# td-kwj-zp2023/webgpu-msm-bls12-377

Hardware: AMD Instinct MI355X
Metric: ms per 2^20 BLS12-377 G1 MSM (lower is better)
Workload: dtype u32 (29-bit limbs, 64-bit accumulate)

## Files before the change

include/msm377.h:

```cpp
#ifndef MSM377_H
#define MSM377_H

#include <stdint.h>

#ifdef __cplusplus
extern "C" {
#endif

#define MSM377_OK 0
#define MSM377_EINVAL (-1)
#define MSM377_EHIP (-2)
#define MSM377_ESCALAR (-3)
#define MSM377_ENOMEM (-4)
#define MSM377_ESTATE (-5)
#define MSM377_EGLVRANGE (-6)
#define MSM377_EEXCEPTIONAL (-7)
#define MSM377_EPOINT (-8)

#define MSM377_NUM_WINDOWS 16
#define MSM377_WINDOW_BITS 16
#define MSM377_G1_PARTIAL_POINTS 16
#define MSM377_G1_POINT_WORDS 48
#define MSM377_G1_WINDOW_PARTIAL_BYTES (MSM377_G1_PARTIAL_POINTS * MSM377_G1_POINT_WORDS * 4)

// ... 141 lines not shown
int msm377_g1_read_mul_table(msm377_ctx* ctx, uint32_t which, uint32_t index, msm377_mul_table_info* info, uint64_t first, uint64_t count, uint32_t* words);

int msm377_g1_xyzz_to_affine(const uint32_t xyzz[52], uint8_t out_xy[96]);

int msm377_ctx_set_glv(msm377_ctx* ctx, int mode);

int msm377_ctx_set_g1_form(msm377_ctx* ctx, int form);

int msm377_ctx_set_narrow_max(msm377_ctx* ctx, uint64_t max_points);

#define MSM377_FB_ACCUMULATE 4
#define MSM377_FB_MERGE 8
#define MSM377_FB_TREE 16
#define MSM377_FB_TAIL 32
#define MSM377_FB_CONVERT 64
int msm377_ctx_get_fallback_info(const msm377_ctx* ctx, uint64_t* count, uint32_t* last_mask);


int msm377_g1_batch_mul_device(msm377_ctx* ctx, const uint8_t base_xy[96], const void* d_scalars, uint64_t n, uint32_t out_form, void* d_out_points, uint8_t* d_out_inf);
int msm377_g1_batch_mul(msm377_ctx* ctx, const uint8_t base_xy[96], const uint8_t* scalars, uint64_t n, uint32_t out_form, uint8_t* out_points, uint8_t* out_inf);
int msm377_g1_batch_mul_host(const uint8_t base_xy[96], const uint8_t* scalars, uint64_t n, uint32_t out_form, uint8_t* out_points, uint8_t* out_inf);
int msm377_ctx_set_mul_window(msm377_ctx* ctx, int window_bits);
int msm377_ctx_get_last_mul_window(const msm377_ctx* ctx);
uint64_t msm377_ctx_get_mul_table_builds(const msm377_ctx* ctx);


#define MSM377_MUL_MAX_BASES 16
int msm377_g1_batch_mul_multi_device(msm377_ctx* ctx, const uint8_t* bases_xy , uint32_t k, const void* d_scalars, uint64_t n, uint64_t out_stride,
                                     uint64_t base_stride, uint32_t out_form, void* d_out_points, uint8_t* d_out_inf);
int msm377_g1_batch_mul_multi(msm377_ctx* ctx, const uint8_t* bases_xy, uint32_t k, const uint8_t* scalars, uint64_t n, uint64_t out_stride, uint64_t base_stride,
                              uint32_t out_form, uint8_t* out_points, uint8_t* out_inf);
int msm377_g1_batch_mul_multi_host(const uint8_t* bases_xy, uint32_t k, const uint8_t* scalars, uint64_t n, uint64_t out_stride, uint64_t base_stride, uint32_t out_form,
                                   uint8_t* out_points, uint8_t* out_inf);
uint64_t msm377_ctx_get_mul_multi_table_builds(const msm377_ctx* ctx);


int msm377_ed_batch_mul_multi_device(msm377_ctx* ctx, const uint8_t* bases_xy , uint32_t k, const void* d_scalars, uint64_t n, uint64_t out_stride,
                                     uint64_t base_stride, void* d_out_points);
int msm377_ed_batch_mul_multi(msm377_ctx* ctx, const uint8_t* bases_xy, uint32_t k, const uint8_t* scalars, uint64_t n, uint64_t out_stride, uint64_t base_stride,
                              uint8_t* out_points);
int msm377_ed_batch_mul_multi_host(const uint8_t* bases_xy, uint32_t k, const uint8_t* scalars, uint64_t n, uint64_t out_stride, uint64_t base_stride, uint8_t* out_points);
uint64_t msm377_ed_ctx_get_mul_table_builds(const msm377_ctx* ctx);
int msm377_ed_read_mul_table(msm377_ctx* ctx, uint32_t index, msm377_mul_table_info* info, uint64_t first, uint64_t count, uint32_t* words);


int msm377_g1_batch_mul_var_device(msm377_ctx* ctx, const void* d_points, const void* d_scalars, uint64_t n, uint32_t scalar_stride, uint32_t out_form, void* d_out_points,
                                   uint8_t* d_out_inf);
int msm377_g1_batch_mul_var(msm377_ctx* ctx, const uint8_t* points, const uint8_t* scalars, uint64_t n, uint32_t scalar_stride, uint32_t out_form, uint8_t* out_points,
                            uint8_t* out_inf);
int msm377_g1_batch_mul_var_host(const uint8_t* points, uint32_t point_form, const uint8_t* scalars, uint32_t scalar_form, uint64_t n, uint32_t scalar_stride,
                                 uint32_t out_form, uint8_t* out_points, uint8_t* out_inf);


int msm377_g1_batch_lincomb2_device(msm377_ctx* ctx, const void* d_p, const void* d_q, const void* d_a, const void* d_b, uint64_t n, uint32_t a_stride, uint32_t b_stride,
                                    uint32_t out_form, void* d_out_points, uint8_t* d_out_inf);
int msm377_g1_batch_lincomb2(msm377_ctx* ctx, const uint8_t* p, const uint8_t* q, const uint8_t* a, const uint8_t* b, uint64_t n, uint32_t a_stride, uint32_t b_stride,
                             uint32_t out_form, uint8_t* out_points, uint8_t* out_inf);
int msm377_g1_batch_lincomb2_host(const uint8_t* p, const uint8_t* q, uint32_t point_form, const uint8_t* a, const uint8_t* b, uint32_t scalar_form, uint64_t n, uint32_t a_stride,
                                  uint32_t b_stride, uint32_t out_form, uint8_t* out_points, uint8_t* out_inf);


#define MSM377_GEN_MAX      4096
#define MSM377_GEN_WIDE_MAX   64
int msm377_g1_set_generators(msm377_ctx* ctx, const uint8_t* gens_xy , uint32_t k, int window_bits);
int msm377_ctx_get_generators(const msm377_ctx* ctx, uint32_t* k, int* window_bits);
int msm377_g1_commit_rows_device(msm377_ctx* ctx, const void* d_scalars, uint64_t n, uint32_t k, uint64_t out_stride, uint64_t base_stride, uint32_t out_form, void* d_out_points,
                                 uint8_t* d_out_inf);
int msm377_g1_commit_rows(msm377_ctx* ctx, const uint8_t* scalars, uint64_t n, uint32_t k, uint64_t out_stride, uint64_t base_stride, uint32_t out_form, uint8_t* out_points,
                          uint8_t* out_inf);
int msm377_g1_commit_rows_host(const uint8_t* gens_xy, uint32_t k, const uint8_t* scalars, uint32_t scalar_form, uint64_t n, uint64_t out_stride, uint64_t base_stride,
                               uint32_t out_form, uint8_t* out_points, uint8_t* out_inf);
void msm377_commit_rows_plan(uint32_t k, uint32_t* segments, uint32_t* bases_per_segment, uint64_t* rows_per_pass);


#define MSM377_STAGE_CONVERT 0
#define MSM377_STAGE_DECOMPOSE 1
#define MSM377_STAGE_SORT 2
#define MSM377_STAGE_ACCUMULATE 3
#define MSM377_STAGE_REDUCE 4
#define MSM377_STAGE_TAIL 5
#define MSM377_STAGE_ACC_KERNEL 6
#define MSM377_NUM_STAGES 7
int msm377_ctx_set_timing(msm377_ctx* ctx, int enabled);
int msm377_ctx_get_stage_ms(msm377_ctx* ctx, double* ms_out);
int msm377_ctx_get_products_per_addition(const msm377_ctx* ctx);

#ifdef __cplusplus
}
#endif
#endif
```

webgpu-msm-bls12-377_amd/csrc/capi.hip:

```cpp
#include <hip/hip_runtime.h>
#include <stdlib.h>
#include <string.h>

#include <algorithm>

#include "context.hpp"
#include "host_tail.hpp"
#include "sequencer.hpp"
#include "batch_mul_host.hpp"
#include "batch_mul_multi_host.hpp"
#include "ed_batch_mul_host.hpp"
#include "commit_rows_host.hpp"
#include "commit_rows_plan.hpp"
#include "batch_lincomb2_host.hpp"
#include "batch_mul_var_host.hpp"
#include "import_host.hpp"
#include "validate_host.hpp"

using namespace msm377;


extern "C" {

const char* msm377_version(void) { return "msm377 0.1 gfx950"; }
// ... 292 lines not shown
  return batch_lincomb2_host(p, q, point_form, a, b, scalar_form, n, a_stride, b_stride, out_form, out_points, out_inf);
}

int msm377_ctx_set_mul_window(msm377_ctx* ctx, int window_bits) {
  if (!ctx || (window_bits != 0 && !batch_mul_width_supported(window_bits))) return MSM377_EINVAL;
  ctx->bm.window = window_bits;
  return MSM377_OK;
}

int msm377_ctx_get_last_mul_window(const msm377_ctx* ctx) { return ctx ? ctx->bm.last_window : 0; }

uint64_t msm377_ctx_get_mul_table_builds(const msm377_ctx* ctx) { return ctx ? ctx->bm.builds : 0; }

uint64_t msm377_ctx_get_mul_multi_table_builds(const msm377_ctx* ctx) { return ctx ? ctx->bmm.builds : 0; }

int msm377_ed_batch_mul_multi_host(const uint8_t* bases_xy, uint32_t k, const uint8_t* scalars, uint64_t n, uint64_t out_stride, uint64_t base_stride, uint8_t* out_points) {
  return ed_batch_mul_multi_host(bases_xy, k, scalars, n, out_stride, base_stride, out_points);
}

uint64_t msm377_ed_ctx_get_mul_table_builds(const msm377_ctx* ctx) { return ctx ? ctx->edbm.builds : 0; }

int msm377_ctx_get_last_check(const msm377_ctx* ctx, msm377_check_report* out) {
  if (!ctx || !out) return MSM377_EINVAL;
  *out = ctx->last_check;
  return MSM377_OK;
}

static int check_host_args(const uint8_t* points, uint64_t n, uint32_t flags, msm377_check_report* out) {
  return (!out || !check_flags_normal(flags) || (n && !points)) ? MSM377_EINVAL : MSM377_OK;
}
int msm377_g1_check_points_host(const uint8_t* points, uint64_t n, uint32_t flags, msm377_check_report* out) {
  if (check_host_args(points, n, flags, out)) return MSM377_EINVAL;
  check_points_host<G1HostCheck>(points, n, check_flags_normal(flags), out);
  return MSM377_OK;
}
int msm377_ed_check_points_host(const uint8_t* points, uint64_t n, uint32_t flags, msm377_check_report* out) {
  if (check_host_args(points, n, flags, out)) return MSM377_EINVAL;
  check_points_host<EdHostCheck>(points, n, check_flags_normal(flags), out);
  return MSM377_OK;
}

uint32_t msm377_short_windows(uint32_t scalar_bits, uint32_t bucket_log) {
  if (scalar_bits < 1 || scalar_bits > 253 || bucket_log < 1 || bucket_log > 15) return 0;
  return short_windows(scalar_bits, bucket_log);
}

int msm377_scalars_width_host(const uint8_t* scalars, uint64_t n, uint32_t scalar_bytes, uint32_t* bits_out) {
  if (!bits_out || (n && !scalars) || (scalar_bytes != 4 && scalar_bytes != 8 && scalar_bytes != 16 && scalar_bytes != 32)) return MSM377_EINVAL;
  uint32_t best = 0;
  for (uint64_t i = 0; i < n; i++) {
    const uint8_t* k = scalars + i * scalar_bytes;
    for (uint32_t j = scalar_bytes; j-- > 0;) {
      if (!k[j]) continue;
      const uint32_t len = 8 * j + 32 - (uint32_t)__builtin_clz((uint32_t)k[j]);
      best = std::max(best, len);
      break;
    }
  }
  *bits_out = best;
  return MSM377_OK;
}

int msm377_ctx_get_last_geometry(const msm377_ctx* ctx, uint32_t* windows, uint32_t* bucket_log) {
  if (!ctx) return MSM377_EINVAL;
  if (windows) *windows = ctx->last.geom_windows;
  if (bucket_log) *bucket_log = ctx->last.geom_log;
  return MSM377_OK;
}

uint32_t msm377_ctx_get_last_sort_elem_bytes(const msm377_ctx* ctx) { return ctx ? ctx->last.sort_elem : 0u; }

int msm377_ctx_set_narrow_max(msm377_ctx* ctx, uint64_t max_points) {
  if (!ctx) return MSM377_EINVAL;
  ctx->knobs.narrow_max_points = max_points;
  return MSM377_OK;
}

int msm377_ctx_set_timing(msm377_ctx* ctx, int enabled) {
  if (!ctx) return MSM377_EINVAL;
  ctx->timing = enabled == 2 ? 2 : (enabled != 0);
  return MSM377_OK;
}

int msm377_ctx_get_stage_ms(msm377_ctx* ctx, double* ms_out) {
  if (!ctx || !ms_out) return MSM377_EINVAL;
  for (int s = 0; s < MSM377_NUM_STAGES; s++) ms_out[s] = ctx->last.stage_ms[s];
  return MSM377_OK;
}

static int ed_wire_only(msm377_ctx* ctx) {
  if (!ctx || (ctx->point_form == MSM377_POINTS_WIRE && ctx->scalar_form == MSM377_SCALARS_WIRE)) return MSM377_OK;
  ctx->err = "the Edwards-BLS12 calls take the wire format only (msm377_ctx_set_input_format)";
  return MSM377_EINVAL;
}
int msm377_ctx_reserve_host_staging(msm377_ctx* ctx) { return eng::reserve_host_staging(ctx); }
int msm377_g1_msm_device(msm377_ctx* ctx, const void* d_points, const void* d_scalars, uint64_t n, uint8_t out_xy[96]) { return converted(ctx, eng::g1_msm_device(ctx, d_points, d_scalars, n, out_xy)); }
int msm377_g1_msm(msm377_ctx* ctx, const uint8_t* points, const uint8_t* scalars, uint64_t n, uint8_t out_xy[96]) { return converted(ctx, eng::g1_msm(ctx, points, scalars, n, out_xy)); }
int msm377_g1_msm_short_device(msm377_ctx* ctx, const void* d_points, const void* d_scalars, uint64_t n, uint32_t scalar_bytes, uint32_t scalar_bits, uint8_t out_xy[96]) { return converted(ctx, eng::g1_msm_short_device(ctx, d_points, d_scalars, n, scalar_bytes, scalar_bits, out_xy)); }
int msm377_g1_msm_short(msm377_ctx* ctx, const uint8_t* points, const uint8_t* scalars, uint64_t n, uint32_t scalar_bytes, uint32_t scalar_bits, uint8_t out_xy[96]) { return converted(ctx, eng::g1_msm_short(ctx, points, scalars, n, scalar_bytes, scalar_bits, out_xy)); }
int msm377_g1_msm_fixed_base_short_device(msm377_ctx* ctx, const void* d_scalars, uint64_t n, uint32_t scalar_bytes, uint32_t scalar_bits, uint8_t out_xy[96]) { return eng::g1_msm_fixed_base_short_device(ctx, d_scalars, n, scalar_bytes, scalar_bits, out_xy); }
int msm377_scalars_width_device(msm377_ctx* ctx, const void* d_scalars, uint64_t n, uint32_t scalar_bytes, uint32_t* bits_out) { return eng::scalars_width_device(ctx, d_scalars, n, scalar_bytes, bits_out); }
int msm377_ed_msm_device(msm377_ctx* ctx, const void* d_points, const void* d_scalars, uint64_t n, uint8_t out_xy[64]) { return converted(ctx, ed_wire_only(ctx) ? MSM377_EINVAL : eng::ed_msm_device(ctx, d_points, d_scalars, n, out_xy)); }
int msm377_ed_msm(msm377_ctx* ctx, const uint8_t* points, const uint8_t* scalars, uint64_t n, uint8_t out_xy[64]) { return converted(ctx, ed_wire_only(ctx) ? MSM377_EINVAL : eng::ed_msm(ctx, points, scalars, n, out_xy)); }
int msm377_ed_generate_bases_device(msm377_ctx* ctx, uint64_t seed, uint64_t n, void* d_points_out) { return ed_wire_only(ctx) ? MSM377_EINVAL : eng::ed_generate_bases_device(ctx, seed, n, d_points_out); }
int msm377_ed_batch_mul_multi_device(msm377_ctx* ctx, const uint8_t* bases_xy, uint32_t k, const void* d_scalars, uint64_t n, uint64_t out_stride, uint64_t base_stride,
                                     void* d_out_points) {
  return ed_wire_only(ctx) ? MSM377_EINVAL : eng::ed_batch_mul_multi_device(ctx, bases_xy, k, d_scalars, n, out_stride, base_stride, d_out_points);
}
int msm377_ed_batch_mul_multi(msm377_ctx* ctx, const uint8_t* bases_xy, uint32_t k, const uint8_t* scalars, uint64_t n, uint64_t out_stride, uint64_t base_stride, uint8_t* out_points) {
  return ed_wire_only(ctx) ? MSM377_EINVAL : eng::ed_batch_mul_multi(ctx, bases_xy, k, scalars, n, out_stride, base_stride, out_points);
}
int msm377_ed_read_mul_table(msm377_ctx* ctx, uint32_t index, msm377_mul_table_info* info, uint64_t first, uint64_t count, uint32_t* words) {
  return eng::ed_read_mul_table(ctx, index, info, first, count, words);
}
int msm377_g1_set_bases_device(msm377_ctx* ctx, const void* d_points, uint64_t n) { return converted(ctx, eng::g1_set_bases_device(ctx, d_points, n)); }
int msm377_g1_set_bases(msm377_ctx* ctx, const uint8_t* points, uint64_t n) { return converted(ctx, eng::g1_set_bases(ctx, points, n)); }
int msm377_g1_set_bases_precomputed_device(msm377_ctx* ctx, const void* d_points, uint64_t n) { return converted(ctx, eng::g1_set_bases_precomputed_device(ctx, d_points, n)); }
int msm377_g1_set_bases_precomputed(msm377_ctx* ctx, const uint8_t* points, uint64_t n) { return converted(ctx, eng::g1_set_bases_precomputed(ctx, points, n)); }
int msm377_g1_msm_fixed_base_device(msm377_ctx* ctx, const void* d_scalars, uint64_t n, uint8_t out_xy[96]) { return eng::g1_msm_fixed_base_device(ctx, d_scalars, n, out_xy); }
int msm377_g1_msm_fixed_base_batch_device(msm377_ctx* ctx, const void* d_scalars, uint64_t n, uint32_t batch, uint8_t* out_xy) { return eng::g1_msm_fixed_base_batch_device(ctx, d_scalars, n, batch, out_xy); }
int msm377_g1_msm_fixed_base(msm377_ctx* ctx, const uint8_t* scalars, uint64_t n, uint8_t out_xy[96]) { return eng::g1_msm_fixed_base(ctx, scalars, n, out_xy); }
int msm377_g1_glv_window_partials_device(msm377_ctx* ctx, const void* d_points, const void* d_scalars, uint64_t n, uint32_t win_begin, uint32_t win_count, uint8_t* partials_out) { return converted(ctx, eng::g1_glv_window_partials_device(ctx, d_points, d_scalars, n, win_begin, win_count, partials_out)); }
int msm377_g1_generate_bases_device(msm377_ctx* ctx, uint64_t seed, uint64_t n, void* d_points_out) { return eng::g1_generate_bases_device(ctx, seed, n, d_points_out); }
int msm377_g1_batch_mul_device(msm377_ctx* ctx, const uint8_t base_xy[96], const void* d_scalars, uint64_t n, uint32_t out_form, void* d_out_points, uint8_t* d_out_inf) { return eng::g1_batch_mul_device(ctx, base_xy, d_scalars, n, out_form, d_out_points, d_out_inf); }
int msm377_g1_batch_mul(msm377_ctx* ctx, const uint8_t base_xy[96], const uint8_t* scalars, uint64_t n, uint32_t out_form, uint8_t* out_points, uint8_t* out_inf) { return eng::g1_batch_mul(ctx, base_xy, scalars, n, out_form, out_points, out_inf); }
int msm377_g1_batch_mul_multi_device(msm377_ctx* ctx, const uint8_t* bases_xy, uint32_t k, const void* d_scalars, uint64_t n, uint64_t out_stride, uint64_t base_stride,
                                     uint32_t out_form, void* d_out_points, uint8_t* d_out_inf) {
  return eng::g1_batch_mul_multi_device(ctx, bases_xy, k, d_scalars, n, out_stride, base_stride, out_form, d_out_points, d_out_inf);
}
int msm377_g1_batch_mul_multi(msm377_ctx* ctx, const uint8_t* bases_xy, uint32_t k, const uint8_t* scalars, uint64_t n, uint64_t out_stride, uint64_t base_stride, uint32_t out_form,
                              uint8_t* out_points, uint8_t* out_inf) {
  return eng::g1_batch_mul_multi(ctx, bases_xy, k, scalars, n, out_stride, base_stride, out_form, out_points, out_inf);
}
int msm377_g1_set_generators(msm377_ctx* ctx, const uint8_t* gens_xy, uint32_t k, int window_bits) { return eng::g1_set_generators(ctx, gens_xy, k, window_bits); }
int msm377_g1_commit_rows_device(msm377_ctx* ctx, const void* d_scalars, uint64_t n, uint32_t k, uint64_t out_stride, uint64_t base_stride, uint32_t out_form, void* d_out_points,
                                 uint8_t* d_out_inf) {
  return eng::g1_commit_rows_device(ctx, d_scalars, n, k, out_stride, base_stride, out_form, d_out_points, d_out_inf);
}
int msm377_g1_commit_rows(msm377_ctx* ctx, const uint8_t* scalars, uint64_t n, uint32_t k, uint64_t out_stride, uint64_t base_stride, uint32_t out_form, uint8_t* out_points,
                          uint8_t* out_inf) {
  return eng::g1_commit_rows(ctx, scalars, n, k, out_stride, base_stride, out_form, out_points, out_inf);
}
int msm377_g1_batch_mul_var_device(msm377_ctx* ctx, const void* d_points, const void* d_scalars, uint64_t n, uint32_t scalar_stride, uint32_t out_form, void* d_out_points, uint8_t* d_out_inf) {
  return eng::g1_batch_mul_var_device(ctx, d_points, d_scalars, n, scalar_stride, out_form, d_out_points, d_out_inf);
}
int msm377_g1_batch_mul_var(msm377_ctx* ctx, const uint8_t* points, const uint8_t* scalars, uint64_t n, uint32_t scalar_stride, uint32_t out_form, uint8_t* out_points, uint8_t* out_inf) {
  return eng::g1_batch_mul_var(ctx, points, scalars, n, scalar_stride, out_form, out_points, out_inf);
}
int msm377_g1_batch_lincomb2_device(msm377_ctx* ctx, const void* d_p, const void* d_q, const void* d_a, const void* d_b, uint64_t n, uint32_t a_stride, uint32_t b_stride,
                                    uint32_t out_form, void* d_out_points, uint8_t* d_out_inf) {
  return eng::g1_batch_lincomb2_device(ctx, d_p, d_q, d_a, d_b, n, a_stride, b_stride, out_form, d_out_points, d_out_inf);
}
int msm377_g1_batch_lincomb2(msm377_ctx* ctx, const uint8_t* p, const uint8_t* q, const uint8_t* a, const uint8_t* b, uint64_t n, uint32_t a_stride, uint32_t b_stride,
                             uint32_t out_form, uint8_t* out_points, uint8_t* out_inf) {
  return eng::g1_batch_lincomb2(ctx, p, q, a, b, n, a_stride, b_stride, out_form, out_points, out_inf);
}
int msm377_g1_check_points_device(msm377_ctx* ctx, const void* d_points, uint64_t n, uint32_t flags, msm377_check_report* out) { return eng::g1_check_points_device(ctx, d_points, n, flags, out); }
int msm377_g1_check_points(msm377_ctx* ctx, const uint8_t* points, uint64_t n, uint32_t flags, msm377_check_report* out) { return eng::g1_check_points(ctx, points, n, flags, out); }
int msm377_ed_check_points_device(msm377_ctx* ctx, const void* d_points, uint64_t n, uint32_t flags, msm377_check_report* out) { return ed_wire_only(ctx) ? MSM377_EINVAL : eng::ed_check_points_device(ctx, d_points, n, flags, out); }
int msm377_ed_check_points(msm377_ctx* ctx, const uint8_t* points, uint64_t n, uint32_t flags, msm377_check_report* out) { return ed_wire_only(ctx) ? MSM377_EINVAL : eng::ed_check_points(ctx, points, n, flags, out); }

}
```

webgpu-msm-bls12-377_amd/csrc/common.hpp:

```cpp
#pragma once
#include <stdint.h>

#include "../../include/msm377.h"

#ifndef MSM_HD
#if defined(__HIPCC__)
#include <hip/hip_runtime.h>
#define MSM_HD __host__ __device__ __forceinline__
#else
#define MSM_HD inline __attribute__((always_inline))
#endif
#endif

namespace msm377 {

constexpr uint32_t NB = 32768;
constexpr uint32_t NBIN = NB + 1;
constexpr uint32_t RP = NBIN + 1;
constexpr uint32_t PT_WORDS = 52;
constexpr uint32_t BKT_WORDS = 64;
constexpr uint32_t MAX_SORT_BLOCKS = 256;
constexpr uint32_t TREE_LEVELS = 15;
constexpr uint32_t SEG_MIN = 16;
constexpr uint32_t SEG_MAX = 128;
constexpr uint32_t SEG_BINS = SEG_MAX + 1;
constexpr int ERR_SCALAR = 1, ERR_GLV_RANGE = 2, ERR_NARROW_RANGE = 128;
constexpr int ERR_SHORT_WIDTH = 256;
constexpr int ERR_TE_EXCEPTIONAL = MSM377_FB_ACCUMULATE, ERR_TE_MERGE = MSM377_FB_MERGE, ERR_TE_TREE = MSM377_FB_TREE, ERR_TE_CONVERT = MSM377_FB_CONVERT;
constexpr int ERR_TE_ANY = ERR_TE_EXCEPTIONAL | ERR_TE_MERGE | ERR_TE_TREE | ERR_TE_CONVERT;
constexpr uint32_t NARROW_LOG = 11;
constexpr uint32_t NARROW_SEG = 8;
constexpr uint32_t NARROW_EVEN_WINDOWS = 22, NARROW_EVEN_SIGNED = 11, NARROW_EVEN_BITS = NARROW_LOG + 1;
static_assert(NARROW_EVEN_SIGNED * NARROW_EVEN_BITS + (NARROW_EVEN_WINDOWS - NARROW_EVEN_SIGNED) * NARROW_LOG == 253, "the windows cover a 253-bit scalar");
constexpr uint32_t MAX_WINDOW_SLOTS = NARROW_EVEN_WINDOWS > MSM377_NUM_WINDOWS ? NARROW_EVEN_WINDOWS : MSM377_NUM_WINDOWS;

constexpr uint32_t short_windows(uint32_t bits, uint32_t L) { return bits / (L + 1) + 1; }
static_assert(short_windows(253, 15) == MSM377_NUM_WINDOWS && short_windows(253, NARROW_LOG) == NARROW_EVEN_WINDOWS, "at full width: the window counts of the main and the narrow path");

constexpr uint32_t NRANGE = 256;
constexpr uint32_t KRANGE = NB / NRANGE;
constexpr uint32_t KEY_TRACKED = 0x80000000u;
constexpr uint32_t KEY_UNSIGNED = 0x40000000u;
constexpr uint32_t SMALL_SORT_MAX = 1u << 16;
constexpr uint32_t SMALL_BINS_MAX = (1u << 12) + 1;
struct SortElem {
  uint32_t idx_sign;
  uint32_t key;
};
struct SortElem4 {
  uint32_t v;
};
constexpr uint32_t SORT_IDX_BITS = 23, SORT_SUB_BITS = 8;
constexpr uint64_t SORT_PACKED_MAX_COLUMNS = 1ull << SORT_IDX_BITS;
static_assert(SORT_IDX_BITS + SORT_SUB_BITS + 1 == 32, "index, sub and sign fill the 32-bit element");
static_assert(KRANGE < (1u << SORT_SUB_BITS), "sub = 0..KRANGE fits its field");
MSM_HD SortElem4 sort_pack(uint32_t idx, uint32_t sign, uint32_t sub) { return SortElem4{(sign << 31) | (sub << SORT_IDX_BITS) | idx}; }
MSM_HD uint32_t sort_sub(SortElem4 e) { return (e.v >> SORT_IDX_BITS) & ((1u << SORT_SUB_BITS) - 1u); }
MSM_HD uint32_t sort_idx_sign(SortElem4 e) { return e.v & ~(((1u << SORT_SUB_BITS) - 1u) << SORT_IDX_BITS); }
MSM_HD uint32_t range_first_key(uint32_t rg, uint32_t shift) { return rg * (KRANGE >> shift); }
inline uint32_t sort_elem_bytes(uint64_t columns, bool wide) { return (!wide && columns <= SORT_PACKED_MAX_COLUMNS) ? 4u : 8u; }

struct WorkItem {
  uint32_t row;
  uint32_t seg;
};
constexpr uint32_t META_BLOCK_WORDS = 2 * SEG_BINS + 4 + MSM377_NUM_WINDOWS;
constexpr size_t SLOT_WORDS = (size_t)MAX_WINDOW_SLOTS * MSM377_G1_PARTIAL_POINTS * MSM377_G1_POINT_WORDS;

constexpr uint32_t AFF_THREADS = 256, AFF_K = 8, AFF_BLOCK_POINTS = AFF_THREADS * AFF_K;
constexpr uint32_t AFF_STASH_WORDS = 52;
inline uint32_t affine_blocks(uint64_t n) { return (uint32_t)((n + AFF_BLOCK_POINTS - 1) / AFF_BLOCK_POINTS); }

constexpr uint32_t ACC_FLAG_WORD = 4;
constexpr uint32_t EVEN_FROM = 13;
constexpr uint32_t even_offset(uint32_t w) { return 16 * w - (w > EVEN_FROM ? w - EVEN_FROM : 0u); }
static_assert(even_offset(13) == 208 && even_offset(14) == 223 && even_offset(15) == 238 && even_offset(16) == 253, "13 x 16 + 3 x 15 = 253 bits");
constexpr uint32_t WIDE_BITS = MSM377_WIDE_WINDOW_BITS;
constexpr uint32_t WIDE_LOG = 19;
constexpr uint32_t WIDE_WINDOWS = 13;
constexpr uint32_t WIDE_FULL = 6;
constexpr uint32_t wide_width(uint32_t w) { return w < WIDE_FULL ? WIDE_BITS : WIDE_BITS - 1; }
constexpr uint32_t wide_offset(uint32_t w) { return w <= WIDE_FULL ? WIDE_BITS * w : WIDE_BITS * WIDE_FULL + (WIDE_BITS - 1) * (w - WIDE_FULL); }
static_assert(wide_offset(WIDE_WINDOWS - 1) == 234 && wide_offset(WIDE_WINDOWS - 1) + wide_width(WIDE_WINDOWS - 1) == 253, "the windows cover a 253-bit scalar");
constexpr uint32_t WIDE_NRANGE = 4096;
constexpr uint32_t WIDE_POINTS = WIDE_LOG + 1;
static_assert((1u << WIDE_LOG) == WIDE_NRANGE * KRANGE, "ranges of KRANGE keys cover the wide bucket set");
static_assert((1u << WIDE_LOG) <= MSM377_NUM_WINDOWS * NB, "the wide bucket set fits the main path's bucket, row and work-list buffers");
static_assert(WIDE_POINTS * 1 <= MAX_WINDOW_SLOTS * MSM377_G1_PARTIAL_POINTS, "the wide window record fits a partial-record slot");

constexpr uint32_t G1_REC_WORDS = 32;
constexpr uint32_t GLV_WINDOWS = MSM377_GLV_WINDOWS;

}
```

webgpu-msm-bls12-377_amd/csrc/context.hip:

```cpp
#include "context.hpp"

#include <string.h>

#include <algorithm>
#include <new>

#include "sequencer.hpp"

using namespace msm377;

hipError_t Resources::alloc(void** p, size_t bytes) {
  const hipError_t rc = hipMalloc(p, bytes);
  if (rc == hipSuccess) device.push_back(*p);
  else *p = nullptr;
  return rc;
}
hipError_t Resources::alloc_pinned(void** p, size_t bytes, unsigned flags) {
  const hipError_t rc = hipHostMalloc(p, bytes, flags);
  if (rc == hipSuccess) pinned.push_back(*p);
  else *p = nullptr;
  return rc;
}
hipError_t Resources::event(hipEvent_t* e, unsigned flags) {
  const hipError_t rc = hipEventCreateWithFlags(e, flags);
// ... 15 lines not shown
}
void Resources::release_all() {
  for (void* p : device) (void)hipFree(p);
  for (void* p : pinned) (void)hipHostFree(p);
  for (hipEvent_t e : events) (void)hipEventDestroy(e);
  for (auto s = streams.rbegin(); s != streams.rend(); ++s) (void)hipStreamDestroy(*s);
  *this = Resources();
}

bool WideBuffers::ensure(Resources& own, uint64_t n, size_t counts_words) {
  if (cap >= n) return true;
  release(own);
  if (own.alloc((void**)&digits, (size_t)WIDE_WINDOWS * n * 4) == hipSuccess && own.alloc((void**)&temp, (size_t)WIDE_WINDOWS * n * sizeof(SortElem)) == hipSuccess &&
      own.alloc((void**)&counts, counts_words * 4) == hipSuccess) {
    cap = n;
    return true;
  }
  release(own);
  (void)hipGetLastError();
  return false;
}
void WideBuffers::release(Resources& own) {
  for (void* p : {(void*)digits, (void*)temp, (void*)counts}) own.release(p);
  *this = WideBuffers();
}

namespace msm377 {
namespace eng {

int ctx_create(int device, uint64_t max_points, const Knobs& knobs, bool borrows_bases, msm377_ctx** out) {
  if (!out || max_points == 0 || max_points > (1ull << 30)) return MSM377_EINVAL;
  *out = nullptr;
  int count = 0;
  if (hipGetDeviceCount(&count) != hipSuccess || device < 0 || device >= count) return MSM377_EHIP;
  msm377_ctx* ctx = new (std::nothrow) msm377_ctx();
  if (!ctx) return MSM377_ENOMEM;
  ctx->device = device;
  ctx->cap = ctx->native.cap = max_points;
  ctx->knobs = knobs;
  ctx->tail_pool.wait_limit_ns = (int64_t)knobs.tail_wait_ms * 1000000ll;
  ctx->tail_pool.numa_local = knobs.tail_numa;
  Resources& own = ctx->own;
  const uint64_t cap = max_points;
  int prio_least = 0, prio_greatest = 0;
  bool ok = hipSetDevice(device) == hipSuccess;
  if (ok && hipDeviceGetStreamPriorityRange(&prio_least, &prio_greatest) != hipSuccess) prio_least = prio_greatest = 0;
  ok = ok && own.stream(&ctx->stream, &prio_greatest) == hipSuccess && own.stream(&ctx->stream2, &prio_least) == hipSuccess &&
       own.event(&ctx->bases_ready, hipEventDisableTiming) == hipSuccess;
  auto dalloc = [&](void** p, size_t bytes) { ok = ok && own.alloc(p, bytes) == hipSuccess; };
  if (!borrows_bases) dalloc((void**)&ctx->d_raw_points, cap * 96);
  dalloc((void**)&ctx->d_raw_scalars, cap * 32);
  if (!borrows_bases) dalloc((void**)&ctx->d_bases, 2 * cap * G1_REC_WORDS * 4);
  const uint64_t wcap = std::max<uint64_t>((uint64_t)MSM377_NUM_WINDOWS * cap, (uint64_t)NARROW_EVEN_WINDOWS * std::min<uint64_t>(cap, SMALL_SORT_MAX));
  dalloc((void**)&ctx->d_digits, wcap * 2);
  dalloc((void**)&ctx->d_range_counts, (size_t)NRANGE * MAX_SORT_BLOCKS * 4);
  dalloc((void**)&ctx->d_region_base, (size_t)MSM377_NUM_WINDOWS * (NRANGE + 1) * 4);
  dalloc((void**)&ctx->d_sort_temp, cap * MSM377_NUM_WINDOWS * sizeof(SortElem));
  dalloc((void**)&ctx->d_row_ptr, (size_t)MSM377_NUM_WINDOWS * RP * 4);
  dalloc((void**)&ctx->d_val_idx, wcap * 4);
  dalloc((void**)&ctx->d_buckets, (size_t)MSM377_NUM_WINDOWS * BKT_WORDS * NB * 4);
  dalloc((void**)&ctx->d_partials, (size_t)2 * SLOT_WORDS * 4);
  const uint64_t extra_items = std::max<uint64_t>((uint64_t)MSM377_NUM_WINDOWS * cap / SEG_MIN, (uint64_t)NARROW_EVEN_WINDOWS * std::min<uint64_t>(cap, SMALL_SORT_MAX) / NARROW_SEG) + 2;
  dalloc((void**)&ctx->d_work, ((size_t)MSM377_NUM_WINDOWS * NB + extra_items) * sizeof(WorkItem));
  dalloc((void**)&ctx->d_work_meta, (size_t)META_BLOCK_WORDS * 4);
  dalloc((void**)&ctx->d_row_ovf_base, (size_t)MSM377_NUM_WINDOWS * NB * 4);
  dalloc((void**)&ctx->d_split_rows, (size_t)MSM377_NUM_WINDOWS * NB * 4);
  dalloc((void**)&ctx->d_ovf, (size_t)extra_items * BKT_WORDS * 4);
  AffineConvert& aff = ctx->aff;
  ZeroCopyOut& zc = ctx->zc;
  const size_t aff_blocks = (size_t)affine_blocks(cap) + 1;
  dalloc((void**)&aff.d_count, 64);
  ok = ok && hipMemset(aff.d_count, 0, 64) == hipSuccess;
  dalloc((void**)&aff.d_stash, (size_t)affine_blocks(cap) * AFF_BLOCK_POINTS * AFF_STASH_WORDS * 4);
  dalloc((void**)&aff.d_trees, aff_blocks * 2 * AFF_THREADS * 13 * 4);
  const unsigned host_flags = hipHostMallocMapped | hipHostMallocCoherent;
  ok = ok && own.alloc_pinned((void**)&aff.h_prod, aff_blocks * 48, host_flags) == hipSuccess &&
       own.alloc_pinned((void**)&aff.h_inv, aff_blocks * 48, host_flags) == hipSuccess &&
       own.alloc_pinned((void**)&aff.h_flag, 64, host_flags) == hipSuccess &&
       hipHostGetDevicePointer((void**)&aff.dm_prod, aff.h_prod, 0) == hipSuccess &&
       hipHostGetDevicePointer((void**)&aff.dm_inv, aff.h_inv, 0) == hipSuccess &&
       hipHostGetDevicePointer((void**)&aff.dm_flag, aff.h_flag, 0) == hipSuccess &&
       own.event(&aff.up_done, hipEventDisableTiming) == hipSuccess;
  if (ok) aff.scratch.resize(aff_blocks);
  dalloc((void**)&ctx->d_err, 4 * sizeof(int));
  ok = ok && own.alloc_pinned((void**)&ctx->h_partials, (size_t)2 * SLOT_WORDS * 4, host_flags) == hipSuccess &&
       hipHostGetDevicePointer((void**)&zc.dm_partials, ctx->h_partials, 0) == hipSuccess &&
       own.alloc_pinned((void**)&zc.h_flag, 64, host_flags) == hipSuccess &&
       hipHostGetDevicePointer((void**)&zc.dm_flag, zc.h_flag, 0) == hipSuccess;
  if (ok) memset(zc.h_flag, 0, 64);
  dalloc((void**)&zc.d_count, 64);
  ok = ok && hipMemset(zc.d_count, 0, 64) == hipSuccess;
  ok = ok && own.alloc_pinned((void**)&ctx->h_err, 2 * sizeof(int)) == hipSuccess;
  for (int k = 0; ok && k < 2; k++) ok = ok && own.event(&ctx->done_ev[k], hipEventDisableTiming) == hipSuccess;
  for (int s = 0; ok && s < MSM377_NUM_STAGES; s++)
    for (int k = 0; k < 2; k++) ok = ok && own.event(&ctx->ev[s][k]) == hipSuccess;
  if (!ok) {
    ctx_destroy(ctx);
    return MSM377_ENOMEM;
  }
  *out = ctx;
  return MSM377_OK;
}

void ctx_destroy(msm377_ctx* ctx) {
  if (!ctx) return;
  ctx->tail_pool.shutdown();
  (void)hipSetDevice(ctx->device);
  if (ctx->stream) (void)hipStreamSynchronize(ctx->stream);
  if (ctx->stream2) (void)hipStreamSynchronize(ctx->stream2);
  if (ctx->twin) {
    twin_return(ctx);
    ctx_destroy(ctx->twin);
    ctx->twin = nullptr;
  }
  ctx->own.release_all();
  delete ctx;
}

int set_stage_capture(msm377_ctx* ctx, int enabled) {
  if (!ctx || enabled < 0 || enabled > 2) return MSM377_EINVAL;
  if (enabled && !ctx->d_buckets_snap) {
    HIP_TRY(ctx, hipSetDevice(ctx->device));
    if (ctx->own.alloc((void**)&ctx->d_buckets_snap, (size_t)MSM377_NUM_WINDOWS * BKT_WORDS * NB * 4) != hipSuccess) return MSM377_ENOMEM;
  }
  ctx->capture = enabled;
  ctx->last.stage.valid = false;
  return MSM377_OK;
}

int reserve_host_staging(msm377_ctx* ctx) {
  if (!ctx) return MSM377_EINVAL;
  HostStaging& st = ctx->staging;
  if (st.h_stage) return MSM377_OK;
  HIP_TRY(ctx, hipSetDevice(ctx->device));
  if (ctx->own.alloc_pinned((void**)&st.h_stage, (size_t)ctx->cap * 128) != hipSuccess) {
    ctx->err = "host staging buffer: out of pinned memory";
    return MSM377_ENOMEM;
  }
  for (int t = 0; t < 8; t++)
    if (!st.copy_stream[t]) HIP_TRY(ctx, ctx->own.stream(&st.copy_stream[t]));
  return MSM377_OK;
}

int ensure_import_buffers(msm377_ctx* ctx, bool host_staging) {
  NativeImport& nat = ctx->native;
  if (!nat.import_done) HIP_TRY(ctx, ctx->own.event(&nat.import_done, hipEventDisableTiming));
  if (!nat.d_inf_mask && ctx->own.alloc((void**)&nat.d_inf_mask, (2 * nat.mask_words() + 4) * 4) != hipSuccess) {
    (void)hipGetLastError();
    ctx->err = "native input forms: out of device memory";
    return MSM377_ENOMEM;
  }
  if (host_staging && !nat.d_native && ctx->own.alloc((void**)&nat.d_native, nat.points_bytes() + (size_t)ctx->cap * 32) != hipSuccess) {
    (void)hipGetLastError();
    ctx->err = "native input forms: out of device memory for the host-buffer staging";
    return MSM377_ENOMEM;
  }
  return MSM377_OK;
}

int bm_alloc(msm377_ctx* ctx, uint32_t** p, size_t bytes) {
  if (*p) return MSM377_OK;
  if (ctx->own.alloc((void**)p, bytes) != hipSuccess) {
    (void)hipGetLastError();
    ctx->err = "out of device memory for the batch multiplication scratch";
    return MSM377_ENOMEM;
  }
  return MSM377_OK;
}

}
}
```

webgpu-msm-bls12-377_amd/csrc/context.hpp:

```cpp
#pragma once
#include <hip/hip_runtime.h>

#include <functional>
#include <string>
#include <vector>

#include "common.hpp"
#include "fp64_host.hpp"
#include "knobs.hpp"
#include "tail_pool.hpp"

using msm377::SortElem;
using msm377::WorkItem;
using msm377::TailPool;
using msm377::Fp64;
using msm377::MAX_WINDOW_SLOTS;
using msm377::NARROW_SEG;
using msm377::Knobs;

struct Resources {
  std::vector<void*> device, pinned;
  std::vector<hipEvent_t> events;
  std::vector<hipStream_t> streams;
  hipError_t alloc(void** p, size_t bytes);
// ... 26 lines not shown
  int width = 0;
  uint32_t* table = nullptr;
  uint64_t table_cap = 0;
};

struct BatchMulState {
  int window = 0;
  int last_window = 0;
  uint64_t builds = 0;
  MulTableSlot single;
  uint32_t* stash = nullptr;
  uint32_t* trees = nullptr;
  uint32_t* block_prod = nullptr;
  uint32_t* block_inv = nullptr;
  uint32_t* row_bases = nullptr;
  uint32_t* base_wire = nullptr;
  uint32_t* var_table = nullptr;
};

struct BatchMulMultiState {
  MulTableSlot slot[MSM377_MUL_MAX_BASES];
  uint64_t builds = 0;
  uint32_t* row_bases = nullptr;
  uint32_t* bases_wire = nullptr;
};

struct EdBatchMulState {
  MulTableSlot slot[MSM377_MUL_MAX_BASES];
  uint64_t builds = 0;
};

struct GeneratorSet {
  uint32_t k = 0;
  int width = 0;
  uint32_t* tables = nullptr;
  bool valid() const { return k != 0; }
};

struct WideBuffers {
  uint32_t* digits = nullptr;
  SortElem* temp = nullptr;
  uint32_t* counts = nullptr;
  uint64_t cap = 0;
  bool ensure(Resources& own, uint64_t n, size_t counts_words);
  void release(Resources& own);
};

struct StageLayout {
  bool valid = false;
  msm377_stage_info info = {};
  const void* d_digits = nullptr;
  const uint32_t* d_key_max = nullptr;
  uint32_t coord_words = 16, limbs = 13;
};

struct BasesLayout {
  bool valid = false;
  msm377_bases_info info = {};
  const uint32_t* d_records = nullptr;
  const uint32_t* d_flagged = nullptr;
};


struct AffineConvert {
  uint32_t* d_stash = nullptr;
  uint32_t* d_trees = nullptr;
  uint32_t* h_prod = nullptr;
  uint32_t* h_inv = nullptr;
  uint32_t* h_flag = nullptr;
  uint32_t *dm_prod = nullptr, *dm_inv = nullptr, *dm_flag = nullptr;
  uint32_t* d_count = nullptr;
  hipEvent_t up_done = nullptr;
  std::vector<Fp64::El> scratch;
};

struct ZeroCopyOut {
  bool active = false;
  uint32_t out_seq = 0;
  uint32_t acc_seq = 0;
  uint32_t* h_flag = nullptr;
  uint32_t* dm_flag = nullptr;
  uint32_t* dm_partials = nullptr;
  uint32_t* d_count = nullptr;
};

struct NativeImport {
  uint64_t cap = 0;
  uint8_t* d_native = nullptr;
  uint32_t* d_inf_mask = nullptr;
  hipEvent_t import_done = nullptr;
  size_t mask_words() const { return (size_t)(((cap + 31) / 32 + 3) & ~3ull); }
  size_t points_bytes() const { return ((size_t)cap * 104 + 15) & ~(size_t)15; }
  uint8_t* native_points() const { return d_native; }
  uint8_t* native_scalars() const { return d_native + points_bytes(); }
};

struct HostStaging {
  uint8_t* h_stage = nullptr;
  hipStream_t copy_stream[8] = {};
};

struct LastCall {
  uint64_t n = 0;
  uint32_t geom_windows = 0, geom_log = 0;
  uint32_t sort_elem = 0;
  int form = -1;
  bool glv = false;
  int products = 0;
  double stage_ms[MSM377_NUM_STAGES] = {};
  StageLayout stage;
  BasesLayout bases;
};

struct Fallbacks {
  uint64_t count = 0;
  uint32_t mask = 0;
  uint64_t geometry_reruns = 0;
};

struct msm377_ctx {
  int device = 0;
  Resources own;
  Knobs knobs;
  hipStream_t stream = nullptr;
  hipStream_t stream2 = nullptr;
  hipEvent_t bases_ready = nullptr;
  uint64_t cap = 0;
  std::string err;
  uint32_t* d_raw_points = nullptr;
  uint32_t* d_raw_scalars = nullptr;
  uint32_t* d_bases = nullptr;
  uint16_t* d_digits = nullptr;
  uint32_t* d_range_counts = nullptr;
  uint32_t* d_region_base = nullptr;
  SortElem* d_sort_temp = nullptr;
  uint32_t* d_row_ptr = nullptr;
  uint32_t* d_val_idx = nullptr;
  uint32_t* d_buckets = nullptr;
  uint32_t* d_buckets_snap = nullptr;
  uint32_t* d_partials = nullptr;
  WorkItem* d_work = nullptr;
  uint32_t* d_work_meta = nullptr;
  uint32_t* d_row_ovf_base = nullptr;
  uint32_t* d_split_rows = nullptr;
  uint32_t* d_ovf = nullptr;
  int* d_err = nullptr;
  uint32_t* h_partials = nullptr;
  int* h_err = nullptr;
  hipEvent_t done_ev[2] = {};
  hipEvent_t ev[MSM377_NUM_STAGES][2] = {};
  uint32_t point_form = MSM377_POINTS_WIRE, scalar_form = MSM377_SCALARS_WIRE;
  int capture = 0;
  int timing = 0;
  ResidentBases resident;
  BatchMulState bm;
  BatchMulMultiState bmm;
  EdBatchMulState edbm;
  GeneratorSet gens;
  WideBuffers wide;
  AffineConvert aff;
  ZeroCopyOut zc;
  NativeImport native;
  HostStaging staging;
  LastCall last;
  Fallbacks fallback;
  msm377_check_report last_check = {0, 0, 0, 0, UINT64_MAX, 0, 0};
  std::function<int()> before_accumulate;
  TailPool tail_pool;
  msm377_ctx* twin = nullptr;
  bool twin_failed = false;
};

namespace msm377 {
namespace eng {

int ctx_create(int device, uint64_t max_points, const Knobs& knobs, bool borrows_bases, msm377_ctx** out);
void ctx_destroy(msm377_ctx* ctx);
int set_stage_capture(msm377_ctx* ctx, int enabled);
int reserve_host_staging(msm377_ctx* ctx);
int ensure_import_buffers(msm377_ctx* ctx, bool host_staging);
int bm_alloc(msm377_ctx* ctx, uint32_t** p, size_t bytes);

}
}
```

webgpu-msm-bls12-377_amd/csrc/kernels/accumulate.hpp:

```cpp
#pragma once
#include "../curves.hpp"
#include "reduce.hpp"

namespace msm377 {
namespace {



__device__ __forceinline__ const uint32_t* row_bounds(const uint32_t* __restrict__ row_ptr, uint32_t L, uint32_t ws, uint32_t t) {
  return row_ptr + (size_t)ws * ((1u << L) + 2) + t + 1;
}
__device__ __forceinline__ uint32_t row_len(const uint32_t* __restrict__ row_ptr, uint32_t L, uint32_t row) {
  const int at = (int)(row + 2 * (row >> L) + 1);
  return row_ptr[at + 1] - row_ptr[at];
}

struct RowSplit {
  uint32_t nseg, seglen, lastlen;
};
__device__ __forceinline__ RowSplit row_split(uint32_t len, uint32_t SEG) {
  RowSplit r;
  if (len <= SEG) {
    r.nseg = 1;
    r.seglen = r.lastlen = len;
    return r;
  }
  const uint32_t parts = (len + SEG - 1) / SEG;
  r.seglen = (len + parts - 1) / parts;
  r.nseg = (len + r.seglen - 1) / r.seglen;
  r.lastlen = len - (r.nseg - 1) * r.seglen;
  return r;
}

__global__ void __launch_bounds__(1024) k_work_hist(const uint32_t* __restrict__ row_ptr, uint32_t L, uint32_t rows, uint32_t SEG, uint32_t* __restrict__ work_hist,
                                                   uint32_t* __restrict__ row_ovf_base, uint32_t* __restrict__ counters ,
                                                   uint32_t* __restrict__ split_rows) {
  __shared__ uint32_t lh[SEG_BINS];
  __shared__ uint32_t blk[4];
  const uint32_t tid = threadIdx.x, row = blockIdx.x * 1024 + tid;
  if (tid < SEG_BINS) lh[tid] = 0;
  if (tid < 2) blk[tid] = 0;
  __syncthreads();
  RowSplit sp = {1, 0, 0};
  uint32_t my_split = 0, my_ovf = 0;
  if (row < rows) {
    sp = row_split(row_len(row_ptr, L, row), SEG);
    atomicAdd(&lh[sp.lastlen], 1u);
    if (sp.nseg > 1) {
      atomicAdd(&lh[sp.seglen], sp.nseg - 1);
      my_split = atomicAdd(&blk[0], 1u);
      my_ovf = atomicAdd(&blk[1], sp.nseg - 1);
    }
  }
  __syncthreads();
  if (tid < SEG_BINS && lh[tid]) atomicAdd(&work_hist[tid], lh[tid]);
  if (tid == 0 && blk[0]) {
    blk[2] = atomicAdd(&counters[0], blk[0]);
    blk[3] = atomicAdd(&counters[1], blk[1]);
  }
  __syncthreads();
  if (sp.nseg > 1) {
    row_ovf_base[row] = blk[3] + my_ovf;
    split_rows[blk[2] + my_split] = row;
  }
}

__global__ void __launch_bounds__(1024) k_work_scatter(const uint32_t* __restrict__ row_ptr, uint32_t L, uint32_t rows, uint32_t SEG,
                                                      const uint32_t* __restrict__ work_hist, uint32_t* __restrict__ cursor, uint32_t* __restrict__ total,
                                                      WorkItem* __restrict__ work) {
  __shared__ uint32_t lh[SEG_BINS];
  __shared__ uint32_t lbase[SEG_BINS];
  __shared__ uint32_t gh[SEG_BINS];
  const uint32_t tid = threadIdx.x, row = blockIdx.x * 1024 + tid;
  if (tid < SEG_BINS) {
    lh[tid] = 0;
    gh[tid] = work_hist[tid];
  }
  __syncthreads();
  uint32_t first = 0;
  if (tid < SEG_BINS) {
    for (uint32_t b = tid + 1; b < SEG_BINS; b++) first += gh[b];
    if (tid == 0 && blockIdx.x == 0) *total = first + gh[0];
  }
  RowSplit sp = {0, 0, 0};
  uint32_t rank_full = 0, rank_last = 0;
  if (row < rows) {
    sp = row_split(row_len(row_ptr, L, row), SEG);
    if (sp.nseg > 1) rank_full = atomicAdd(&lh[sp.seglen], sp.nseg - 1);
    rank_last = atomicAdd(&lh[sp.lastlen], 1u);
  }
  __syncthreads();
  if (tid < SEG_BINS && lh[tid]) lbase[tid] = first + atomicAdd(&cursor[tid], lh[tid]);
  __syncthreads();
  if (row < rows) {
    for (uint32_t s = 0; s + 1 < sp.nseg; s++) work[lbase[sp.seglen] + rank_full + s] = WorkItem{row, s};
    work[lbase[sp.lastlen] + rank_last] = WorkItem{row, sp.nseg - 1};
  }
}

template <class T>
__device__ __forceinline__ void pin_registers(T& o) {
  static_assert(sizeof(T) % 4 == 0, "whole words");
  uint32_t w[sizeof(T) / 4];
  __builtin_memcpy(w, &o, sizeof(T));
#pragma unroll
  for (int j = 0; j < (int)(sizeof(T) / 4); j++) asm volatile("" : "+v"(w[j]));
  __builtin_memcpy(&o, w, sizeof(T));
}

template <class CV, int OCC, class BP = CV, int PF = 0>
__global__ void __launch_bounds__(256, OCC) k_accumulate(const uint32_t* __restrict__ row_ptr, const uint32_t* __restrict__ val_idx,
                                                       const uint32_t* __restrict__ bases, uint32_t* __restrict__ buckets, uint64_t n,
                                                       const WorkItem* __restrict__ work, const uint32_t* __restrict__ work_total,
                                                       const uint32_t* __restrict__ row_ovf_base, uint32_t* __restrict__ ovf, uint32_t SEG,
                                                       int* __restrict__ err, const int* __restrict__ conv_err, uint32_t into, uint64_t table_stride, uint32_t L) {
  const uint32_t v = blockIdx.x * 256 + threadIdx.x;
  if (v == 0 && *conv_err) atomicOr(err, *conv_err);
  if (v >= *work_total) return;
  const WorkItem it = work[v];
  const uint32_t ws = it.row >> L, t = it.row & ((1u << L) - 1);
  const uint32_t* rb = row_bounds(row_ptr, L, ws, t);
  const uint32_t* vi = val_idx + (size_t)ws * n;
  bases += (size_t)ws * table_stride * BP::REC_WORDS;
  const uint32_t row_beg = rb[0], row_end = rb[1];
  const uint32_t seglen = row_split(row_end - row_beg, SEG).seglen;
  uint32_t k = row_beg + it.seg * seglen;
  const uint32_t end = (row_end - k > seglen) ? k + seglen : row_end;
  typename CV::Pt acc = (into && it.seg == 0) ? load_bucket<CV>(buckets, L, ws, t) : CV::identity();
  const bool start_fresh = !(into && it.seg == 0);
  bool bad = false;
  if (k < end) {
    static_assert(PF == 0, "one record in flight");
    uint32_t e_cur = vi[k];
    uint32_t e_nxt = (k + 1 < end) ? vi[k + 1] : 0u;
    typename BP::Base rec = BP::load_base(bases, e_cur & 0x7fffffffu);
    bool more = true;
    auto advance = [&]() {
      k++;
      more = k < end;
      if (more) {
        rec = BP::load_base(bases, e_nxt & 0x7fffffffu);
        e_cur = e_nxt;
        e_nxt = (k + 1 < end) ? vi[k + 1] : 0u;
      }
    };
    auto stage = [&](auto first_tag) {
      constexpr bool FIRST = decltype(first_tag)::value;
      const bool neg = (e_cur >> 31) != 0;
      if constexpr (FIRST) {
        const typename BP::Base cur = rec;
        advance();
        acc = BP::first(cur, neg);
      } else {
        typename BP::Ops ops = BP::signed_ops(rec, neg);
        pin_registers(ops);
        advance();
        acc = BP::madd(acc, ops);
      }
      bad |= CV::is_bad(acc);
    };
    if (start_fresh) stage(std::true_type{});
    while (more) stage(std::false_type{});
  }
  if (bad) atomicOr(err, ERR_TE_EXCEPTIONAL);
  if (it.seg == 0) {
    store_bucket<CV>(buckets, L, ws, t, acc);
  } else {
    store_record<CV>(ovf + (size_t)(row_ovf_base[it.row] + it.seg - 1) * CV::BKT_WORDS, acc);
  }
}

template <class F, class K>
__device__ __forceinline__ typename TeLazy<F, K>::Ext te_madd_quad(const typename TeLazy<F, K>::Ext& a, const typename F::El& mine, uint32_t q) {
  using El = typename F::El;
  const El m1 = F::mul_lz(sel4(q, F::add_kp_sub(a.y, K::KP2, a.x), F::add_lz(a.y, a.x), a.t, a.z), mine);
  const El pa = quad_bcast<0>(m1), pb = quad_bcast<1>(m1), c = quad_bcast<2>(m1), d = quad_bcast<3>(m1);
  const El e = F::norm(F::add_kp_sub(pb, K::KP2, pa)), f = F::norm(F::add_kp_sub(d, K::KP2, c));
  const El g = F::norm(F::add_lz(d, c)), h = F::add_lz(pb, pa);
  const El m3 = F::mul_lz(sel4(q, e, h, h, f), sel4(q, f, g, e, g));
  typename TeLazy<F, K>::Ext o;
  o.x = quad_bcast<0>(m3);
  o.y = quad_bcast<1>(m3);
  o.t = quad_bcast<2>(m3);
  o.z = quad_bcast<3>(m3);
  return o;
}

template <class CV>
__global__ void __launch_bounds__(256, 2) k_accumulate_quad(const uint32_t* __restrict__ row_ptr, const uint32_t* __restrict__ val_idx,
                                                          const uint32_t* __restrict__ bases, uint32_t* __restrict__ buckets, uint64_t n,
                                                          const WorkItem* __restrict__ work, const uint32_t* __restrict__ work_total,
                                                          const uint32_t* __restrict__ row_ovf_base, uint32_t* __restrict__ ovf, uint32_t SEG,
                                                          int* __restrict__ err, const int* __restrict__ conv_err, uint32_t into, uint32_t L) {
  using El = typename CV::F::El;
  using K = typename CV::Pt_K;
  const uint32_t gid = blockIdx.x * 256 + threadIdx.x;
  const uint32_t v = gid >> 2, q = threadIdx.x & 3;
  if (gid == 0 && *conv_err) atomicOr(err, *conv_err);
  if (v >= *work_total) return;
  const WorkItem it = work[v];
  const uint32_t ws = it.row >> L, t = it.row & ((1u << L) - 1);
  const uint32_t* rb = row_bounds(row_ptr, L, ws, t);
  const uint32_t* vi = val_idx + (size_t)ws * n;
  const uint32_t row_beg = rb[0], row_end = rb[1];
  const uint32_t seglen = row_split(row_end - row_beg, SEG).seglen;
  uint32_t k = row_beg + it.seg * seglen;
  const uint32_t end = (row_end - k > seglen) ? k + seglen : row_end;
  const bool continues = into && it.seg == 0;
  typename CV::Pt acc = continues ? load_bucket<CV>(buckets, L, ws, t) : CV::identity();
  bool bad = false;
  auto load_mine = [&](uint32_t e) {
    const bool neg = (e >> 31) != 0;
    const uint32_t comp = q < 2 ? (q ^ (neg ? 1u : 0u)) : q;
    const uint32_t* src = bases + (size_t)(e & 0x7fffffffu) * CV::REC_WORDS + comp * CV::NL;
    El r;
#pragma unroll
    for (int j = 0; j < (int)CV::NL; j++) r.l[j] = src[j];
    return r;
  };
  if (k < end && !continues) {
    const uint32_t e = vi[k];
    acc = CV::first(CV::load_base(bases, e & 0x7fffffffu), (e >> 31) != 0);
    bad |= CV::is_bad(acc);
    k++;
  }
  if (k < end) {
    uint32_t e_cur = vi[k];
    uint32_t e_nxt = (k + 1 < end) ? vi[k + 1] : 0u;
    El cur = load_mine(e_cur);
    for (;;) {
      k++;
      const bool more = k < end;
      El nxt = cur;
      uint32_t e_nn = 0u;
      if (more) {
        nxt = load_mine(e_nxt);
        if (k + 1 < end) e_nn = vi[k + 1];
      }
      const El mine = (q == 2 && (e_cur >> 31)) ? CV::F::kp_sub(K::KP2, cur) : cur;
      acc = te_madd_quad<typename CV::F, K>(acc, mine, q);
      bad |= CV::is_bad(acc);
      if (!more) break;
      cur = nxt;
      e_cur = e_nxt;
      e_nxt = e_nn;
    }
  }
  if (bad) atomicOr(err, ERR_TE_EXCEPTIONAL);
  uint32_t* dst = it.seg == 0 ? bucket_ptr<CV>(buckets, L, ws, t) : ovf + (size_t)(row_ovf_base[it.row] + it.seg - 1) * CV::BKT_WORDS;
  store_coord<CV>(dst + q * CV::COORD_WORDS, coord4(q, acc).l);
}

constexpr uint32_t OVF_FOLDED = 0x80000000u;
constexpr uint32_t LONG_ROW_PARTIALS = 32, FOLD_THREADS = 512, FOLD_BLOCKS = 64;
static_assert((1u << 15) <= FOLD_THREADS * FOLD_BLOCKS, "one pass of the grid sees every row of a window (L <= 15)");
template <class CV>
__global__ void __launch_bounds__(FOLD_THREADS) k_fold_long_rows(const uint32_t* __restrict__ row_ptr, uint32_t* __restrict__ row_ovf_base, uint32_t* __restrict__ ovf,
                                                                 uint32_t SEG, int* __restrict__ err, uint32_t L, uint32_t ws) {
  __shared__ uint32_t list[FOLD_THREADS];
  __shared__ uint32_t nlist;
  if (threadIdx.x == 0) nlist = 0;
  __syncthreads();
  {
    const uint32_t t = blockIdx.x + gridDim.x * threadIdx.x;
    if (t < (1u << L) && row_split(row_len(row_ptr, L, (ws << L) + t), SEG).nseg > LONG_ROW_PARTIALS) list[atomicAdd(&nlist, 1u)] = (ws << L) + t;
  }
  __syncthreads();
  const uint32_t q = threadIdx.x & 3, quad = threadIdx.x >> 2;
  bool bad = false;
  for (uint32_t i = 0; i < nlist; i++) {
    const uint32_t row = list[i];
    uint32_t* rec = ovf + (size_t)row_ovf_base[row] * CV::BKT_WORDS;
    for (uint32_t cur = row_split(row_len(row_ptr, L, row), SEG).nseg - 1; cur > 1;) {
      const uint32_t half = (cur + 1) / 2;
      for (uint32_t j = quad; j + half < cur; j += FOLD_THREADS / 4) {
        uint32_t* a = rec + (size_t)j * CV::BKT_WORDS;
        const typename CV::Pt sum = add_quad(load_record_quad<CV>(a, q), load_record_quad<CV>(rec + (size_t)(j + half) * CV::BKT_WORDS, q), q);
        bad |= CV::is_bad(sum);
        store_coord<CV>(a + q * CV::COORD_WORDS, coord4(q, sum).l);
      }
      cur = half;
      __syncthreads();
    }
  }
  __syncthreads();
  for (uint32_t i = threadIdx.x; i < nlist; i += FOLD_THREADS) row_ovf_base[list[i]] |= OVF_FOLDED;
  if (bad) atomicOr(err, ERR_TE_MERGE);
}

template <class CV>
__global__ void __launch_bounds__(256, 2) k_merge_split_rows_quad(const uint32_t* __restrict__ row_ptr, uint32_t* __restrict__ buckets,
                                                                  const uint32_t* __restrict__ counters, const uint32_t* __restrict__ split_rows,
                                                                  const uint32_t* __restrict__ row_ovf_base, const uint32_t* __restrict__ ovf, uint32_t SEG,
                                                                  int* __restrict__ err, uint32_t L, uint32_t* __restrict__ host_flag, uint32_t seq) {
  if (host_flag && blockIdx.x == 0 && threadIdx.x == 0) __hip_atomic_store(host_flag, seq, __ATOMIC_RELAXED, __HIP_MEMORY_SCOPE_SYSTEM);
  const uint32_t count = counters[0];
  const uint32_t q = threadIdx.x & 3;
  for (uint32_t i = (blockIdx.x * 256 + threadIdx.x) >> 2; i < count; i += gridDim.x * 64) {
    const uint32_t row = split_rows[i];
    const uint32_t len = row_len(row_ptr, L, row);
    const uint32_t ovf_at = row_ovf_base[row];
    const uint32_t nseg = (ovf_at & OVF_FOLDED) ? 2u : row_split(len, SEG).nseg;
    const uint32_t ws = row >> L, t = row & ((1u << L) - 1);
    typename CV::Pt acc = load_bucket_quad<CV>(buckets, L, ws, t, q);
    const uint32_t* src = ovf + (size_t)(ovf_at & ~OVF_FOLDED) * CV::BKT_WORDS;
    typename CV::Pt nxt = load_record_quad<CV>(src, q);
    bool bad = false;
    for (uint32_t s = 1; s < nseg; s++) {
      const typename CV::Pt cur = nxt;
      if (s + 1 < nseg) nxt = load_record_quad<CV>(src + (size_t)s * CV::BKT_WORDS, q);
      acc = add_quad(acc, cur, q);
      bad |= CV::is_bad(acc);
    }
    if (bad) atomicOr(err, ERR_TE_MERGE);
    const typename CV::F::El c = coord4(q, acc);
    store_coord<CV>(bucket_ptr<CV>(buckets, L, ws, t) + q * CV::COORD_WORDS, c.l);
  }
}

}
}
```

webgpu-msm-bls12-377_amd/csrc/kernels/sort.hpp:

```cpp
#pragma once
#include "../curves.hpp"
#include "decompose.hpp"

namespace msm377 {
namespace {



template <class F>
__device__ __forceinline__ void for_each_digit(const uint16_t* __restrict__ dg, uint64_t beg, uint64_t end, uint32_t tid, uint32_t nthreads, F f) {
  uint64_t head = beg;
  while (head < end && (((uintptr_t)(dg + head)) & 15)) head++;
  for (uint64_t i = beg + tid; i < head; i += nthreads) f(i, (uint32_t)dg[i]);
  const uint64_t groups = (end - head) / 8;
  const uint4* v = reinterpret_cast<const uint4*>(dg + head);
  for (uint64_t g = tid; g < groups; g += nthreads) {
    const uint4 q = v[g];
    const uint32_t w[4] = {q.x, q.y, q.z, q.w};
#pragma unroll
    for (int k = 0; k < 4; k++) {
      f(head + g * 8 + 2 * k, w[k] & 0xffffu);
      f(head + g * 8 + 2 * k + 1, w[k] >> 16);
    }
  }
// ... 88 lines not shown
    cnt[tid] = 0;
  }
  __syncthreads();
  const uint64_t beg = (uint64_t)c * per_chunk;
  const uint64_t end = (beg + per_chunk < n) ? beg + per_chunk : n;
  const uint16_t* dg = digits + (size_t)ws * n;
  E* out = temp + (size_t)ws * n;
  for (uint64_t tile0 = beg; tile0 < end; tile0 += PT_TILE) {
    const uint64_t i0 = tile0 + (uint64_t)tid * 8;
    uint32_t d[8];
    uint32_t valid = 0;
    if (i0 + 8 <= end && (((uintptr_t)(dg + i0)) & 15) == 0) {
      const uint4 q = *reinterpret_cast<const uint4*>(dg + i0);
      const uint32_t w[4] = {q.x, q.y, q.z, q.w};
#pragma unroll
      for (int k = 0; k < 4; k++) {
        d[2 * k] = w[k] & 0xffffu;
        d[2 * k + 1] = w[k] >> 16;
      }
      valid = 0xffu;
    } else {
#pragma unroll
      for (int j = 0; j < 8; j++) {
        d[j] = 0;
        if (i0 + j < end) {
          d[j] = dg[i0 + j];
          valid |= 1u << j;
        }
      }
    }
    uint32_t key[8], sign[8], rg[8], rk[8];
#pragma unroll
    for (int j = 0; j < 8; j++) {
      digit_key(d[j], uns, key[j], sign[j]);
      rg[j] = key_range(key[j], shift);
      rk[j] = 0;
      if ((valid >> j) & 1u) rk[j] = atomicAdd(&cnt[rg[j]], 1u);
    }
    __syncthreads();
    uint32_t mine = 0, incl = 0;
    if (tid < NRANGE) {
      mine = cnt[tid];
      incl = mine;
#pragma unroll
      for (int off = 1; off < 64; off <<= 1) {
        const uint32_t v = __shfl_up((int)incl, off, 64);
        if ((tid & 63) >= (uint32_t)off) incl += v;
      }
      if ((tid & 63) == 63) wsum[tid >> 6] = incl;
    }
    __syncthreads();
    if (tid < NRANGE) {
      uint32_t before = 0;
      for (uint32_t w = 0; w < (tid >> 6); w++) before += wsum[w];
      const uint32_t excl = before + incl - mine;
      toff[tid] = excl;
      gdelta[tid] = cur[tid] - excl;
      cur[tid] += mine;
      cnt[tid] = 0;
    }
    __syncthreads();
#pragma unroll
    for (int j = 0; j < 8; j++)
      if ((valid >> j) & 1u) {
        const uint32_t slot = toff[rg[j]] + rk[j];
        stage[slot] = Ops::make((uint32_t)(i0 + j), sign[j], key[j], rg[j], shift);
        if constexpr (Ops::TAGGED) tag[slot] = (uint8_t)rg[j];
      }
    __syncthreads();
    const uint32_t tile_len = (uint32_t)((end - tile0 < PT_TILE) ? end - tile0 : PT_TILE);
    for (uint32_t p = tid; p < tile_len; p += 1024) {
      const E e = stage[p];
      uint32_t range;
      if constexpr (Ops::TAGGED)
        range = tag[p];
      else
        range = key_range(e.key, shift);
      out[gdelta[range] + p] = e;
    }
    __syncthreads();
  }
}

constexpr uint32_t LS_CACHE = 6144;
constexpr uint32_t LS_REG = LS_CACHE / 256;
template <class E>
__global__ void __launch_bounds__(256) k_local_sort_lds(const E* __restrict__ temp, const uint32_t* __restrict__ region_base,
                                                        uint32_t* __restrict__ row_ptr, uint32_t* __restrict__ val_idx, uint64_t n,
                                                        const uint32_t* __restrict__ key_max, uint32_t NR, uint32_t NBK) {
  using Ops = ElemOps<E>;
  constexpr uint32_t NBINS = KRANGE + 1;
  static_assert(NBINS <= 256, "one bin per thread");
  __shared__ uint32_t bins[NBINS];
  __shared__ uint32_t part[256];
  __shared__ uint32_t sorted[LS_CACHE];
  const uint32_t RPW = NBK + 2;
  const uint32_t r = blockIdx.x, ws = blockIdx.y, tid = threadIdx.x;
  const uint32_t shift = key_max ? win_shift(key_max[ws]) : 0u;
  const uint32_t KR = KRANGE >> shift;
  const uint32_t lo = r * KR;
  const bool last = shift == 0 && r == NR - 1;
  const uint32_t nb = KR + (last ? 1u : 0u);
  const uint32_t rbeg = region_base[ws * (NR + 1) + r], rend = region_base[ws * (NR + 1) + r + 1];
  const uint32_t len = rend - rbeg;
  const bool cached = len <= LS_CACHE;
  const E* in = temp + (size_t)ws * n + rbeg;
  if (tid < NBINS) bins[tid] = 0;
  __syncthreads();
  E e[LS_REG];
  if (cached) {
#pragma unroll
    for (uint32_t u = 0; u < LS_REG; u++) {
      const uint32_t i = u * 256 + tid;
      e[u] = Ops::none(lo);
      if (i < len) e[u] = in[i];
    }
#pragma unroll
    for (uint32_t u = 0; u < LS_REG; u++)
      if (u * 256 + tid < len) atomicAdd(&bins[Ops::bin(e[u], lo)], 1u);
  } else {
    for (uint32_t i0 = 0; i0 < len; i0 += 2048) {
      E f[8];
#pragma unroll
      for (int u = 0; u < 8; u++) {
        const uint32_t i = i0 + u * 256 + tid;
        f[u] = Ops::none(lo);
        if (i < len) f[u] = in[i];
      }
#pragma unroll
      for (int u = 0; u < 8; u++)
        if (i0 + u * 256 + tid < len) atomicAdd(&bins[Ops::bin(f[u], lo)], 1u);
    }
  }
  __syncthreads();
  const uint32_t own = tid < nb ? bins[tid] : 0u;
  part[tid] = own;
  __syncthreads();
  for (uint32_t off = 1; off < 256; off <<= 1) {
    const uint32_t v = tid >= off ? part[tid - off] : 0u;
    __syncthreads();
    part[tid] += v;
    __syncthreads();
  }
  uint32_t* rp = row_ptr + (size_t)ws * RPW + lo;
  const uint32_t start = rbeg + part[tid] - own;
  __syncthreads();
  if (tid < nb) {
    bins[tid] = start;
    rp[tid] = start;
  }
  if (tid == 0 && last) rp[nb] = rend;
  if (shift) {
    const uint32_t covered = NR * KR, total = region_base[ws * (NR + 1) + NR];
    const uint32_t per_block = (RPW - covered + NR - 1) / NR;
    uint32_t* rp_w = row_ptr + (size_t)ws * RPW;
    for (uint32_t j = tid; j < per_block; j += 256) {
      const uint32_t idx = covered + r * per_block + j;
      if (idx < RPW) rp_w[idx] = total;
    }
  }
  __syncthreads();
  uint32_t* vi = val_idx + (size_t)ws * n;
  if (cached) {
#pragma unroll
    for (uint32_t u = 0; u < LS_REG; u++)
      if (u * 256 + tid < len) sorted[atomicAdd(&bins[Ops::bin(e[u], lo)], 1u) - rbeg] = Ops::idx_sign(e[u]);
    __syncthreads();
    for (uint32_t i = tid; i < len; i += 256) vi[rbeg + i] = sorted[i];
  } else {
    for (uint32_t i0 = 0; i0 < len; i0 += 2048) {
      E f[8];
#pragma unroll
      for (int u = 0; u < 8; u++) {
// ... 64 lines not shown
```

webgpu-msm-bls12-377_amd/csrc/knobs.hpp:

```cpp
#pragma once
#include <limits.h>
#include <stdint.h>
#include <stdlib.h>

#include <algorithm>
#include <type_traits>
#include <utility>

#include "common.hpp"
#include "tail_pool.hpp"
#include "validate_host.hpp"

namespace msm377 {

struct Knobs {
  int glv_mode = 0;
  int g1_form = 1;
  uint32_t conv_wave_prio = 1;
  int64_t aff_prewake_us = 600;
  uint32_t upload_chunks = 4;
  uint32_t upload_split_pct = 30;
  uint64_t upload_chunk_min = 1ull << 18;
  int tail_threads = 6;
  int tail_wait_ms = 2000;
  int64_t tail_spin_us = 1000;
  bool tail_trace = false;
  bool tail_numa = true;
  bool te_affine_msm = true;
  uint64_t narrow_max_points = 1ull << 16;
  int precomp_bits = MSM377_WINDOW_BITS;
  uint64_t affine_min_points = 1ull << 20;
  uint32_t seg_plain = 0, seg_glv = 0;
  int zc_out = 1;
  uint32_t narrow_seg = 0;
  uint64_t narrow_quad_items = 100000;
  uint32_t coop_threads = 131072;
  uint32_t narrow_tail_from = 4;
  bool tail_lds = true;
  bool reduce_columns = true;
  bool even_windows = true;
  uint32_t sort_elem = 8;
  bool twin_batches = true;
  uint32_t base_checks = 0;
  uint32_t tail_from = 7;

  static inline Knobs from_env();
};

namespace knob_rule {
template <auto F>
using field_t = std::remove_reference_t<decltype(std::declval<Knobs&>().*F)>;
template <auto F>
void flag(Knobs& k, const char* e) { k.*F = atoi(e) != 0; }
template <auto F>
void raw_int(Knobs& k, const char* e) { k.*F = (field_t<F>)atoi(e); }
template <auto F, int LO, int HI>
void int_in(Knobs& k, const char* e) { k.*F = (field_t<F>)std::min(std::max(atoi(e), LO), HI); }
template <auto F>
void u64(Knobs& k, const char* e) { k.*F = strtoull(e, nullptr, 10); }
template <auto F>
void i64(Knobs& k, const char* e) { k.*F = atoll(e); }
inline void wide_or_16(Knobs& k, const char* e) { k.precomp_bits = atoi(e) == (int)WIDE_BITS ? (int)WIDE_BITS : MSM377_WINDOW_BITS; }
inline void four_or_8(Knobs& k, const char* e) { k.sort_elem = atoi(e) == 4 ? 4u : 8u; }
inline void check_mask(Knobs& k, const char* e) { k.base_checks = check_flags_normal((uint32_t)strtoul(e, nullptr, 0)); }
}

inline Knobs Knobs::from_env() {
  using namespace knob_rule;
  static constexpr struct {
    const char* name;
    void (*rule)(Knobs&, const char*);
  } TABLE[] = {
      {"MSM377_GLV", raw_int<&Knobs::glv_mode>},
      {"MSM377_G1_FORM", flag<&Knobs::g1_form>},
      {"MSM377_CONV_WAVE_PRIO", flag<&Knobs::conv_wave_prio>},
      {"MSM377_AFF_PREWAKE_US", i64<&Knobs::aff_prewake_us>},
      {"MSM377_UPLOAD_CHUNKS", int_in<&Knobs::upload_chunks, 2, 7>},
      {"MSM377_UPLOAD_SPLIT", int_in<&Knobs::upload_split_pct, 5, 90>},
      {"MSM377_UPLOAD_CHUNK_MIN", u64<&Knobs::upload_chunk_min>},
      {"MSM377_TAIL_THREADS", int_in<&Knobs::tail_threads, 1, TailPool::WORKERS + 1>},
      {"MSM377_TAIL_WAIT_MS", int_in<&Knobs::tail_wait_ms, 1, INT_MAX>},
      {"MSM377_TAIL_SPIN_US", i64<&Knobs::tail_spin_us>},
      {"MSM377_TAIL_TRACE", flag<&Knobs::tail_trace>},
      {"MSM377_TAIL_NUMA", flag<&Knobs::tail_numa>},
      {"MSM377_TE_AFFINE_MSM", flag<&Knobs::te_affine_msm>},
      {"MSM377_NARROW_MAX", u64<&Knobs::narrow_max_points>},
      {"MSM377_PRECOMP_BITS", wide_or_16},
      {"MSM377_AFFINE_MIN", u64<&Knobs::affine_min_points>},
      {"MSM377_SEG_PLAIN", int_in<&Knobs::seg_plain, (int)SEG_MIN, (int)SEG_MAX>},
      {"MSM377_SEG_GLV", int_in<&Knobs::seg_glv, (int)SEG_MIN, (int)SEG_MAX>},
      {"MSM377_ZERO_COPY_OUT", raw_int<&Knobs::zc_out>},
      {"MSM377_NARROW_SEG", int_in<&Knobs::narrow_seg, (int)NARROW_SEG, (int)SEG_BINS - 1>},
      {"MSM377_NARROW_QUAD_ITEMS", u64<&Knobs::narrow_quad_items>},
      {"MSM377_COOP_THREADS", raw_int<&Knobs::coop_threads>},
      {"MSM377_NARROW_TAIL_FROM", int_in<&Knobs::narrow_tail_from, 1, (int)TREE_LEVELS>},
      {"MSM377_TAIL_LDS", flag<&Knobs::tail_lds>},
      {"MSM377_REDUCE_COLUMNS", flag<&Knobs::reduce_columns>},
      {"MSM377_EVEN_WINDOWS", flag<&Knobs::even_windows>},
      {"MSM377_SORT_ELEM", four_or_8},
      {"MSM377_TWIN_BATCH", flag<&Knobs::twin_batches>},
      {"MSM377_BASE_CHECKS", check_mask},
      {"MSM377_TAIL_FROM", int_in<&Knobs::tail_from, 1, (int)TREE_LEVELS>},
  };
  Knobs k;
  for (const auto& row : TABLE)
    if (const char* e = getenv(row.name)) row.rule(k, e);
  return k;
}

}
```

webgpu-msm-bls12-377_amd/csrc/sequencer.hip:

```cpp
#include "sequencer.hpp"

#include <hip/hip_runtime.h>
#include <string.h>

#include <algorithm>
#include <atomic>
#include <chrono>
#include <functional>
#include <initializer_list>
#include <thread>
#include <type_traits>
#include <vector>

#include "context.hpp"
#include "host_tail.hpp"
#include "ed_batch_mul_host.hpp"
#include "validate_host.hpp"
#include "kernels/accumulate.hpp"
#include "kernels/batch_mul.hpp"
#include "kernels/batch_mul_multi.hpp"
#include "kernels/ed_batch_mul.hpp"
#include "kernels/commit_rows.hpp"
#include "kernels/convert.hpp"
#include "kernels/decompose.hpp"
// ... 12 lines not shown
bool hip_ok(msm377_ctx* ctx, int hip_error, const char* what) {
  const hipError_t e = (hipError_t)hip_error;
  if (e == hipSuccess) return true;
  if (ctx) ctx->err = std::string(what) + ": " + hipGetErrorString(e);
  return false;
}

namespace {

void note_fallback(msm377_ctx* ctx, uint32_t mask) {
  ctx->fallback.count++;
  ctx->fallback.mask = mask;
}

struct HipFail {
  hipError_t e = hipSuccess;
  const char* what = "";
  int record(msm377_ctx* ctx, int rc) const {
    hip_ok(ctx, e, what);
    return rc;
  }
};
int h2d_staged(msm377_ctx* ctx, void* d_dst, const uint8_t* src, size_t bytes, size_t stage_off, HipFail* fail = nullptr) {
#define H2D_TRY(call)                \
  do {                               \
    const hipError_t e_ = (call);    \
    if (e_ != hipSuccess) {          \
      if (fail) *fail = {e_, #call}; \
      else hip_ok(ctx, e_, #call);   \
      return MSM377_EHIP;            \
    }                                \
  } while (0)
  constexpr int NT_MAX = 8;
  constexpr int NT = 4;
  constexpr size_t SMALL = 8u << 20, PIECE = 4u << 20;
  if (bytes < SMALL) {
    H2D_TRY(hipMemcpy(d_dst, src, bytes, hipMemcpyHostToDevice));
    return MSM377_OK;
  }
  if (!ctx->staging.h_stage && reserve_host_staging(ctx) != MSM377_OK) {
    (void)hipGetLastError();
    H2D_TRY(hipMemcpy(d_dst, src, bytes, hipMemcpyHostToDevice));
    return MSM377_OK;
  }
  size_t npieces = (bytes + PIECE - 1) / PIECE;
  npieces = (npieces + NT - 1) / NT * NT;
  const size_t piece = ((bytes + npieces - 1) / npieces + 4095) & ~(size_t)4095;
  uint8_t* stage = ctx->staging.h_stage + stage_off;
  hipError_t errs[NT_MAX + 1];
  std::thread workers[NT_MAX];
  const int device = ctx->device;
  std::atomic<size_t> next{0};
  auto copy_pieces = [&, device](int t) {
    hipError_t e = hipSetDevice(device);
    for (;;) {
      const size_t c = next.fetch_add(1, std::memory_order_relaxed);
      const size_t off = c * piece;
      if (c >= npieces || off >= bytes || e != hipSuccess) break;
      const size_t len = (bytes - off < piece) ? bytes - off : piece;
      memcpy(stage + off, src + off, len);
      e = hipMemcpyAsync((uint8_t*)d_dst + off, stage + off, len, hipMemcpyHostToDevice, ctx->staging.copy_stream[t]);
    }
    if (e == hipSuccess) e = hipStreamSynchronize(ctx->staging.copy_stream[t]);
    errs[t] = e;
  };
  for (int t = 0; t <= NT; t++) errs[t] = hipSuccess;
  for (int t = 0; t < NT; t++) workers[t] = std::thread([&copy_pieces, t] { copy_pieces(t); });
  copy_pieces(NT);
  for (int t = 0; t < NT; t++) workers[t].join();
  for (int t = 0; t <= NT; t++) H2D_TRY(errs[t]);
  return MSM377_OK;
#undef H2D_TRY
}

void identity_wire(uint8_t out[96]) {
  memset(out, 0, 96);
  out[48] = 1;
}

struct StageTimer {
  msm377_ctx* c;
  int s;
  hipStream_t st;
  bool on() const { return c->timing == 1 || (c->timing == 2 && s == MSM377_STAGE_ACC_KERNEL); }
  StageTimer(msm377_ctx* ctx, int stage, hipStream_t stream) : c(ctx), s(stage), st(stream) {
    if (on()) (void)hipEventRecord(c->ev[s][0], st);
  }
  ~StageTimer() {
    if (on()) (void)hipEventRecord(c->ev[s][1], st);
  }
};

void note_bases(msm377_ctx* ctx, uint32_t form, const uint32_t* d_records, uint64_t n, uint64_t first = 0, bool glv = false) {
  static const uint32_t REC[4] = {64, 40, 32, 32}, LIMBS[4] = {13, 13, 13, 9}, COORDS[4] = {4, 3, 2, 3};
  BasesLayout b;
  b.info.form = form;
  b.info.record_words = REC[form];
  b.info.limbs = LIMBS[form];
  b.info.coords = COORDS[form];
  b.info.n = first + n;
  b.info.windows = 1;
  b.info.glv = glv ? 1 : 0;
  b.info.window_stride = first + n;
  b.info.records = (glv ? 2 : 1) * (first + n);
  b.d_records = d_records;
  if (form != MSM377_BASES_ED && ctx->point_form == MSM377_POINTS_MONT_FLAG && ctx->native.d_inf_mask) b.d_flagged = ctx->native.d_inf_mask + 2 * ctx->native.mask_words();
  b.valid = true;
  ctx->last.bases = b;
}
template <class CV>
constexpr uint32_t bases_form_of() {
  return std::is_same<CV, TeDev>::value ? MSM377_BASES_TE_PROJECTIVE : std::is_same<CV, EdDev>::value ? MSM377_BASES_ED : MSM377_BASES_WEIERSTRASS;
}

template <class CV>
int convert_bases(msm377_ctx* ctx, const uint32_t* d_raw, uint64_t n, uint64_t first = 0, bool clear_err = true) {
  if (n == 0) return MSM377_OK;
  if (ctx->timing == 1) (void)hipEventRecord(ctx->ev[MSM377_STAGE_CONVERT][0], ctx->stream2);
  if (clear_err) hipLaunchKernelGGL(k_clear_words, dim3(1), dim3(256), 0, ctx->stream2, (uint32_t*)(ctx->d_err + 2), 1u, (uint32_t*)nullptr, 0u);
  hipLaunchKernelGGL(k_convert_bases<CV>, dim3((unsigned)((n + 255) / 256)), dim3(256), 0, ctx->stream2, d_raw, ctx->d_bases + first * CV::REC_WORDS, n,
                     ctx->d_err + 2);
  HIP_TRY(ctx, hipGetLastError());
  note_bases(ctx, bases_form_of<CV>(), ctx->d_bases, n, first);
  if (ctx->timing == 1) (void)hipEventRecord(ctx->ev[MSM377_STAGE_CONVERT][1], ctx->stream2);
  HIP_TRY(ctx, hipEventRecord(ctx->bases_ready, ctx->stream2));
  return MSM377_OK;
}

int affine_convert_begin(msm377_ctx* ctx, const uint32_t* d_raw, uint64_t n, const uint32_t* prev_window_records = nullptr, uint32_t doublings = 0,
                         bool clear_err = true) {
  if (n == 0) return MSM377_OK;
  const uint32_t nblk = affine_blocks(n);
  if (ctx->timing == 1) (void)hipEventRecord(ctx->ev[MSM377_STAGE_CONVERT][0], ctx->stream2);
  __atomic_store_n(ctx->aff.h_flag, 0u, __ATOMIC_RELEASE);
  if (clear_err) hipLaunchKernelGGL(k_clear_words, dim3(1), dim3(256), 0, ctx->stream2, (uint32_t*)(ctx->d_err + 2), 1u, (uint32_t*)nullptr, 0u);
  if (prev_window_records)
    hipLaunchKernelGGL(k_affine_up<AffDoublingSource>, dim3(nblk), dim3(AFF_THREADS), 0, ctx->stream2, AffDoublingSource{prev_window_records, doublings}, n,
                       ctx->aff.d_stash, ctx->aff.d_trees, ctx->aff.dm_prod, ctx->aff.dm_flag, ctx->aff.d_count, ctx->d_err + 2, ctx->knobs.conv_wave_prio);
  else
    hipLaunchKernelGGL(k_affine_up<AffWireSource>, dim3(nblk), dim3(AFF_THREADS), 0, ctx->stream2, AffWireSource{d_raw}, n, ctx->aff.d_stash, ctx->aff.d_trees,
                       ctx->aff.dm_prod, ctx->aff.dm_flag, ctx->aff.d_count, ctx->d_err + 2, ctx->knobs.conv_wave_prio);
  HIP_TRY(ctx, hipGetLastError());
  HIP_TRY(ctx, hipEventRecord(ctx->aff.up_done, ctx->stream2));
  if (ctx->knobs.tail_threads > 1 && nblk >= 32) ctx->tail_pool.prewake(ctx->knobs.aff_prewake_us, std::min(ctx->knobs.tail_threads, TailPool::WORKERS + 1) - 1);
  return MSM377_OK;
}

int affine_convert_finish(msm377_ctx* ctx, uint32_t* d_records_out, uint64_t n) {
  if (n == 0) return MSM377_OK;
  const uint32_t nblk = affine_blocks(n);
  const auto t0 = std::chrono::steady_clock::now();
  for (uint32_t spins = 0; __atomic_load_n(ctx->aff.h_flag, __ATOMIC_ACQUIRE) != nblk; spins++) {
    __builtin_ia32_pause();
    if ((spins & 0xfff) == 0xfff && std::chrono::steady_clock::now() - t0 > std::chrono::milliseconds(20)) {
      HIP_TRY(ctx, hipEventSynchronize(ctx->aff.up_done));
      break;
    }
  }
  if (__atomic_load_n(ctx->aff.h_flag, __ATOMIC_ACQUIRE) != nblk) {
    ctx->err = "batched affine conversion: the block products did not arrive";
    return MSM377_EHIP;
  }
  {
    const int inv_rc = invert_block_products_mt(ctx, 0, nblk);
    ctx->tail_pool.disarm();
    if (inv_rc) return inv_rc;
  }
  hipLaunchKernelGGL(k_affine_down, dim3(nblk), dim3(AFF_THREADS), 0, ctx->stream2, n, ctx->aff.d_stash, ctx->aff.d_trees, ctx->aff.dm_inv, d_records_out, ctx->knobs.conv_wave_prio);
// ... 41 lines not shown
  WindowPlan p = plan_equal16(tail);
  p.recode = RECODE_EVEN16;
  p.short_from = EVEN_FROM;
  return p;
}
WindowPlan plan_narrow22() {
  WindowPlan p = plan_equal16(TE_TAIL, NARROW_EVEN_WINDOWS);
  p.recode = RECODE_NARROW22;
  p.bucket_log = NARROW_LOG;
  p.short_from = NARROW_EVEN_SIGNED;
  return p;
}
WindowPlan folded_behind_table(WindowPlan p, const uint32_t* table, uint64_t stride) {
  p.table = table;
  p.table_stride = stride;
  p.records = 1;
  p.on_caller = true;
  return p;
}
WindowPlan plan_wide13(const uint32_t* table, uint64_t stride) {
  WindowPlan p = folded_behind_table(plan_equal16(TE_TAIL, 1), table, stride);
  p.recode = RECODE_WIDE13;
  p.bucket_log = WIDE_LOG;
  return p;
}
WindowPlan plan_glv8(uint32_t slots = GLV_WINDOWS) {
  WindowPlan p = plan_equal16(XYZZ_TAIL, slots);
  p.recode = RECODE_GLV8;
  p.on_caller = true;
  return p;
}
WindowPlan plan_short(TailKind tail, uint32_t bytes, uint32_t bits, bool narrow) {
  const uint32_t L = narrow ? NARROW_LOG : (uint32_t)MSM377_WINDOW_BITS - 1;
  WindowPlan p = plan_equal16(tail, short_windows(bits, L));
  p.recode = RECODE_SHORT;
  p.bucket_log = L;
  p.short_bytes = bytes;
  p.short_bits = bits;
  return p;
}
WindowPlan plan_whole16(const msm377_ctx* ctx, TailKind tail) { return ctx->knobs.even_windows && tail != XYZZ_TAIL ? plan_even16(tail) : plan_equal16(tail); }

bool geometry_refused(const WindowPlan& p, int err) {
  if (p.recode == RECODE_GLV8) return (err & ERR_GLV_RANGE) != 0;
  const bool can_refuse = p.recode == RECODE_EVEN16 || p.recode == RECODE_NARROW22 || p.recode == RECODE_WIDE13;
  return can_refuse && (err & ERR_NARROW_RANGE) && !(err & ERR_SCALAR);
}
WindowPlan next_plan(const WindowPlan& refused) {
  WindowPlan p = plan_equal16(refused.tail);
  if (refused.recode == RECODE_WIDE13) p.bases_override = refused.table;
  return p;
}

struct Phase {
  bool clear_err = true;
  bool front = true;
  bool into = false;
  bool back = true;
  bool zc_out = false;
  uint64_t base_first = 0;
  WindowPlan plan;
};

struct CurveDims { int form; uint32_t bkt_words, coord_words, limbs, pt_words, out_words, rec_words; bool quad_items; };
template <class CV, class BP>
constexpr CurveDims curve_dims() {
  return {CV::FORM_ID, CV::BKT_WORDS, CV::COORD_WORDS, CV::NL, CV::PT_WORDS, CV::OUT_WORDS, BP::REC_WORDS, std::is_same<BP, CV>::value && std::is_same<CV, TeDev>::value};
}

struct LaunchRecord {
  const WindowPlan& plan;
  CurveDims cv;
  uint32_t into;
  uint64_t n_scalars, n;
  uint32_t wb, slots;
  uint32_t L, buckets, rows;
  uint64_t entries, max_items;
  uint32_t SEG;
  uint32_t wc_out, pp;
  bool narrow, wide, glv, even, is_short, quad_acc, packed_sort;
  uint32_t coop_from, tail_from;
  size_t tail_lds_bytes;
  int* d_err;
  uint32_t* d_partials;
  const uint32_t* bases;
  uint32_t *work_hist, *cursor, *total, *counters;
  uint32_t *key_max, *top_key_max;
};

LaunchRecord launch_record(msm377_ctx* ctx, const Phase& ph, uint64_t n_scalars, uint32_t wb, int slot, const CurveDims& cv) {
  const WindowPlan& plan = ph.plan;
  LaunchRecord k{plan, cv, ph.into ? 1u : 0u};
  k.glv = plan.recode == RECODE_GLV8, k.wide = plan.recode == RECODE_WIDE13, k.even = plan.recode == RECODE_EVEN16, k.is_short = plan.short_bytes != 0;
  k.n_scalars = n_scalars, k.n = k.glv ? 2 * n_scalars : n_scalars, k.wb = wb, k.slots = plan.slots;
  k.L = plan.bucket_log, k.buckets = 1u << k.L;
  k.narrow = !k.wide && k.L != MSM377_WINDOW_BITS - 1;
  k.entries = (k.wide ? (uint64_t)WIDE_WINDOWS : (uint64_t)k.slots) * k.n;
  static_assert((uint64_t)NARROW_EVEN_WINDOWS * SMALL_SORT_MAX / NARROW_SEG + NARROW_EVEN_WINDOWS * (1u << NARROW_LOG) <= (uint64_t)MSM377_NUM_WINDOWS * 32768,
                "narrow work items fit the work-item buffer");
  k.SEG = (k.narrow && !ctx->knobs.seg_plain) ? (ctx->knobs.narrow_seg ? ctx->knobs.narrow_seg : (k.n > 8192 ? 16u : 12u)) : auto_seg(ctx, k.entries, k.glv);
  k.rows = k.slots * k.buckets, k.max_items = (uint64_t)k.rows + k.entries / k.SEG;
  k.wc_out = plan.table ? 1u : k.slots, k.pp = k.wide ? WIDE_POINTS : (uint32_t)MSM377_G1_PARTIAL_POINTS;
  k.quad_acc = cv.quad_items && k.narrow && !plan.table && k.max_items <= ctx->knobs.narrow_quad_items;
  k.packed_sort = !k.wide && !k.narrow && ctx->knobs.sort_elem == 4 && sort_elem_bytes(k.n, false) == 4;
  for (k.coop_from = 0; k.coop_from < k.L && 4ull * (k.coop_from + 1) * (k.buckets >> (k.coop_from + 1)) * k.wc_out > ctx->knobs.coop_threads;) k.coop_from++;
  k.tail_from = std::min(k.wide ? k.L - 8 : k.narrow ? ctx->knobs.narrow_tail_from : ctx->knobs.tail_from, k.L);
  k.tail_lds_bytes = (size_t)(k.buckets >> k.tail_from) * cv.pt_words * 4;
  k.d_err = ctx->d_err + slot, k.d_partials = ctx->d_partials + (size_t)slot * SLOT_WORDS;
  const uint32_t* records = ctx->resident.valid() ? ctx->resident.bases : ctx->d_bases;
  k.bases = plan.table ? plan.table : plan.bases_override ? plan.bases_override : records + ph.base_first * cv.rec_words;
  k.work_hist = ctx->d_work_meta, k.cursor = k.work_hist + SEG_BINS, k.total = k.work_hist + 2 * SEG_BINS, k.counters = k.total + 1;
  k.key_max = k.work_hist + (2 * SEG_BINS + 4);
  const bool measured = k.is_short ? !k.narrow : (!k.glv && !k.even && wb + k.slots == MSM377_NUM_WINDOWS);
  k.top_key_max = measured ? k.key_max + (k.slots - 1) : nullptr;
  return k;
}

int enqueue_decompose(msm377_ctx* ctx, const LaunchRecord& k, const uint32_t* d_scalars) {
  StageTimer t(ctx, MSM377_STAGE_DECOMPOSE, ctx->stream);
  hipStream_t st = ctx->stream;
  const dim3 grid((unsigned)((k.n_scalars + 255) / 256)), block(256);
  const uint32_t bias = k.wide ? 1u << WIDE_LOG : k.narrow ? k.buckets : 1u << (MSM377_WINDOW_BITS - 1);
  const uint32_t top_bias = k.is_short && !k.narrow ? 0u : bias;
  if (k.is_short) {
    const uint32_t sb = k.plan.short_bytes;
    const auto recode = sb == 4 ? k_decompose_short<4> : sb == 8 ? k_decompose_short<8> : sb == 16 ? k_decompose_short<16> : k_decompose_short<32>;
    hipLaunchKernelGGL(recode, grid, block, 0, st, (const uint8_t*)d_scalars, ctx->d_digits, k.n, k.plan.short_bits, k.L, k.slots, bias, top_bias, k.d_err, k.top_key_max);
  } else if (k.wide)
    hipLaunchKernelGGL(k_decompose_wide, grid, block, 0, st, d_scalars, ctx->wide.digits, k.n, k.d_err);
  else if (k.narrow)
    hipLaunchKernelGGL(k_decompose_geom, grid, block, 0, st, d_scalars, ctx->d_digits, k.n, k.L, NARROW_EVEN_SIGNED, k.slots, bias, k.d_err);
  else if (k.glv)
    hipLaunchKernelGGL(k_decompose_glv, grid, block, 0, st, d_scalars, ctx->d_digits, k.n_scalars, k.wb, k.slots, k.d_err);
  else
    hipLaunchKernelGGL(k_decompose, grid, block, 0, st, d_scalars, ctx->d_digits, k.n, k.wb, k.slots, k.d_err, k.top_key_max, k.even ? 1u : 0u);
  HIP_TRY(ctx, hipGetLastError());
  static_assert(MAX_WINDOW_SLOTS <= MSM377_STAGE_MAX_SLOTS, "a stage layout names every window slot");
  msm377_stage_info& info = ctx->last.stage.info = msm377_stage_info{};
  info.slots = k.slots, info.bucket_log = k.L;
  info.columns = k.entries / k.slots;
  info.digit_bytes = k.wide ? 4u : 2u;
  info.row_ptr_len = k.buckets + 2, info.bucket_records = k.buckets;
  info.form = k.cv.form, info.table_stride = k.plan.table_stride, info.geometry_reruns = ctx->fallback.geometry_reruns;
  for (uint32_t s = 0; s < k.slots; s++) info.bias[s] = s + 1 < k.slots ? bias : top_bias;
  if (k.is_short && !k.narrow) info.key_unsigned[k.slots - 1] = 1u;
  ctx->last.stage.d_digits = k.wide ? (const void*)ctx->wide.digits : (const void*)ctx->d_digits;
  ctx->last.stage.d_key_max = (k.wide || k.narrow) ? nullptr : k.key_max;
  ctx->last.stage.coord_words = k.cv.coord_words, ctx->last.stage.limbs = k.cv.limbs;
  return MSM377_OK;
}

int enqueue_sort(msm377_ctx* ctx, const LaunchRecord& k) {
  StageTimer t(ctx, MSM377_STAGE_SORT, ctx->stream);
  hipStream_t st = ctx->stream;
  if (k.wide) {
    uint32_t* counts = ctx->wide.counts;
    ctx->last.sort_elem = sort_elem_bytes(k.entries, true);
    hipLaunchKernelGGL(k_wide_count, dim3(WS_CHUNKS, WIDE_WINDOWS), dim3(1024), 0, st, (const uint32_t*)ctx->wide.digits, counts, k.n);
    hipLaunchKernelGGL(k_wide_sums, dim3(WIDE_NRANGE / 256, WIDE_WINDOWS), dim3(256), 0, st, counts);
    hipLaunchKernelGGL(k_wide_scan, dim3(1), dim3(1024), 0, st, counts, ctx->d_region_base);
    hipLaunchKernelGGL(k_wide_offsets1, dim3(WIDE_WINDOWS), dim3(WS_COARSE), 0, st, counts, k.n);
    hipLaunchKernelGGL(k_wide_part1, dim3(WS_CHUNKS, WIDE_WINDOWS), dim3(1024), 0, st, (const uint32_t*)ctx->wide.digits, (const uint32_t*)counts, ctx->d_sort_temp, k.n, (uint32_t)k.plan.table_stride);
    hipLaunchKernelGGL(k_wide_part2, dim3(WS_COARSE, WIDE_WINDOWS), dim3(1024), 0, st, (const SortElem*)ctx->d_sort_temp, (const uint32_t*)counts, ctx->wide.temp);
    hipLaunchKernelGGL(k_local_sort_lds<SortElem>, dim3(WIDE_NRANGE, 1), dim3(256), 0, st, (const SortElem*)ctx->wide.temp, ctx->d_region_base, ctx->d_row_ptr, ctx->d_val_idx,
                       k.entries, (const uint32_t*)nullptr, WIDE_NRANGE, k.buckets);
    HIP_TRY(ctx, hipGetLastError());
  } else if (k.narrow) {
    ctx->last.sort_elem = 0;
    hipLaunchKernelGGL(k_small_sort, dim3(k.slots), dim3(1024), 0, st, ctx->d_digits, ctx->d_row_ptr, ctx->d_val_idx, (uint32_t)k.n, k.L);
    HIP_TRY(ctx, hipGetLastError());
  } else {
    uint32_t chunks = MAX_SORT_BLOCKS / k.slots;
    const uint64_t want = (k.n + 4095) / 4096;
    if (chunks > want) chunks = (uint32_t)(want ? want : 1);
    const uint64_t per_chunk = (k.n + chunks - 1) / chunks;
    const dim3 grid(chunks, k.slots);
    hipLaunchKernelGGL(k.is_short ? k_range_count<true> : k_range_count<false>, grid, dim3(1024), 0, st, ctx->d_digits, ctx->d_range_counts, k.n, chunks, per_chunk, k.key_max);
    HIP_TRY(ctx, hipGetLastError());
    hipLaunchKernelGGL(k_range_scan, dim3(k.slots), dim3(NRANGE), 0, st, ctx->d_range_counts, ctx->d_region_base, chunks);
    HIP_TRY(ctx, hipGetLastError());
    ctx->last.sort_elem = k.packed_sort ? 4u : 8u;
    auto partition_and_sort = [&](auto* temp) {
      using E = std::remove_pointer_t<decltype(temp)>;
      hipLaunchKernelGGL((k.is_short ? k_partition_staged<E, true> : k_partition_staged<E, false>), grid, dim3(1024), 0, st, ctx->d_digits, ctx->d_range_counts, temp, k.n, chunks,
                         per_chunk, k.key_max);
      const hipError_t e = hipGetLastError();
      if (e != hipSuccess) return e;
      hipLaunchKernelGGL(k_local_sort_lds<E>, dim3(NRANGE, k.slots), dim3(256), 0, st, (const E*)temp, ctx->d_region_base, ctx->d_row_ptr, ctx->d_val_idx, k.n, k.key_max, NRANGE,
                         k.buckets);
      return hipGetLastError();
    };
    HIP_TRY(ctx, k.packed_sort ? partition_and_sort(reinterpret_cast<SortElem4*>(ctx->d_sort_temp)) : partition_and_sort(ctx->d_sort_temp));
  }
  return MSM377_OK;
}

template <class CV, class BP>
void launch_accumulate(msm377_ctx* ctx, const LaunchRecord& k) {
  StageTimer tk(ctx, MSM377_STAGE_ACC_KERNEL, ctx->stream);
  hipStream_t st = ctx->stream;
  if constexpr (curve_dims<CV, BP>().quad_items) {
    if (k.quad_acc) {
      hipLaunchKernelGGL(k_accumulate_quad<CV>, dim3((unsigned)((4 * k.max_items + 255) / 256)), dim3(256), 0, st, ctx->d_row_ptr, ctx->d_val_idx, k.bases, ctx->d_buckets, k.n,
                         ctx->d_work, k.total, ctx->d_row_ovf_base, ctx->d_ovf, k.SEG, k.d_err, ctx->d_err + 2, k.into, k.L);
      return;
    }
  }
  hipLaunchKernelGGL((k_accumulate<CV, 2, BP>), dim3((unsigned)((k.max_items + 255) / 256)), dim3(256), 0, st, ctx->d_row_ptr, ctx->d_val_idx, k.bases, ctx->d_buckets, k.n,
                     ctx->d_work, k.total, ctx->d_row_ovf_base, ctx->d_ovf, k.SEG, k.d_err, ctx->d_err + 2, k.into, k.plan.table_stride, k.L);
}

template <class CV, class BP>
int enqueue_accumulate(msm377_ctx* ctx, const LaunchRecord& k) {
  StageTimer t(ctx, MSM377_STAGE_ACCUMULATE, ctx->stream);
  hipStream_t st = ctx->stream;
  const dim3 row_grid((k.rows + 1023) / 1024);
  hipLaunchKernelGGL(k_work_hist, row_grid, dim3(1024), 0, st, ctx->d_row_ptr, k.L, k.rows, k.SEG, k.work_hist, ctx->d_row_ovf_base, k.counters, ctx->d_split_rows);
  HIP_TRY(ctx, hipGetLastError());
  hipLaunchKernelGGL(k_work_scatter, row_grid, dim3(1024), 0, st, ctx->d_row_ptr, k.L, k.rows, k.SEG, (const uint32_t*)k.work_hist, k.cursor, k.total, ctx->d_work);
  HIP_TRY(ctx, hipGetLastError());
  if (ctx->before_accumulate) {
    std::function<int()> f;
    f.swap(ctx->before_accumulate);
    const int hook_rc = f();
    if (hook_rc) return hook_rc;
  }
  HIP_TRY(ctx, hipStreamWaitEvent(st, ctx->bases_ready, 0));
  ctx->last.products = BP::MADD_PRODUCTS;
  launch_accumulate<CV, BP>(ctx, k);
  HIP_TRY(ctx, hipGetLastError());
  ctx->zc.acc_seq++;
  if (k.is_short) {
    hipLaunchKernelGGL(k_fold_long_rows<CV>, dim3(FOLD_BLOCKS), dim3(FOLD_THREADS), 0, st, ctx->d_row_ptr, ctx->d_row_ovf_base, ctx->d_ovf, k.SEG, k.d_err, k.L, k.slots - 1);
    HIP_TRY(ctx, hipGetLastError());
  }
  hipLaunchKernelGGL(k_merge_split_rows_quad<CV>, dim3(std::min<uint32_t>((k.rows + 63) / 64, 1024u)), dim3(256), 0, st, ctx->d_row_ptr, ctx->d_buckets, k.counters,
                     ctx->d_split_rows, ctx->d_row_ovf_base, ctx->d_ovf, k.SEG, k.d_err, k.L, ctx->zc.dm_flag + ACC_FLAG_WORD, ctx->zc.acc_seq);
  HIP_TRY(ctx, hipGetLastError());
  return MSM377_OK;
}

template <class CV>
int enqueue_reduce(msm377_ctx* ctx, const LaunchRecord& k) {
  static_assert(CV::HAS_QUAD, "every curve policy has the quad-cooperative addition");
  StageTimer t(ctx, MSM377_STAGE_REDUCE, ctx->stream);
  hipStream_t st = ctx->stream;
  for (uint32_t m = k.plan.table ? k.slots : 1; m > 1;) {
    const uint32_t half = (m + 1) / 2, count = m - half;
    hipLaunchKernelGGL(k_fold_windows<CV>, dim3(count * k.buckets / 256), dim3(256), 0, st, ctx->d_buckets, k.L, half, count, k.d_err);
    HIP_TRY(ctx, hipGetLastError());
    m = half;
  }
  uint32_t r = 0;
  while (ctx->knobs.reduce_columns && r < k.tail_from) {
    const uint32_t levels = std::min(k.tail_from - r, COLUMN_LEVELS_MAX);
    const uint32_t threads = (r + 1) * (k.buckets >> (r + 1));
    hipLaunchKernelGGL(k_tree_columns<CV>, dim3((threads + 255) / 256, k.wc_out), dim3(256), 0, st, ctx->d_buckets, k.L, r, levels, k.coop_from, threads, k.d_err);
    HIP_TRY(ctx, hipGetLastError());
    r += levels;
  }
  for (; r < k.tail_from; r++) {
    const uint32_t ops = (r + 1) * (k.buckets >> (r + 1));
    if (r >= k.coop_from)
      hipLaunchKernelGGL(k_tree_step_quad<CV>, dim3((4 * ops + 255) / 256, k.wc_out), dim3(256), 0, st, ctx->d_buckets, k.L, r, ops, k.d_err);
    else
      hipLaunchKernelGGL(k_tree_step<CV>, dim3((ops + 255) / 256, k.wc_out), dim3(256), 0, st, ctx->d_buckets, k.L, r, ops, k.d_err);
    HIP_TRY(ctx, hipGetLastError());
  }
  if (k.tail_from < k.L) {
    const bool in_lds = ctx->knobs.tail_lds && k.tail_lds_bytes <= TAIL_LDS_BYTES_MAX;
    if (in_lds && k.tail_lds_bytes > 64 * 1024)
      HIP_TRY(ctx, hipFuncSetAttribute(reinterpret_cast<const void*>(&k_reduce_tail_lds<CV>), hipFuncAttributeMaxDynamicSharedMemorySize, (int)TAIL_LDS_BYTES_MAX));
    if (in_lds)
      hipLaunchKernelGGL(k_reduce_tail_lds<CV>, dim3(k.tail_from + 1, k.wc_out), dim3(TAIL_THREADS), k.tail_lds_bytes, st, ctx->d_buckets, k.L, k.tail_from, k.d_err);
    else
      hipLaunchKernelGGL(k_reduce_tail<CV>, dim3(k.tail_from + 1, k.wc_out), dim3(TAIL_THREADS), 0, st, ctx->d_buckets, k.L, k.tail_from, k.d_err);
    HIP_TRY(ctx, hipGetLastError());
  }
  const bool zc = ctx->zc.active;
  hipLaunchKernelGGL(k_gather_partials<CV>, dim3((k.wc_out * k.pp * 4 + 63) / 64), dim3(64), 0, st, ctx->d_buckets, k.d_partials, k.wc_out, k.L, zc ? ctx->zc.dm_partials : nullptr,
                     zc ? ctx->zc.dm_flag : nullptr, zc ? ctx->zc.d_count : nullptr, zc ? (const int*)k.d_err : nullptr, zc ? ctx->zc.out_seq : 0u, k.pp);
  HIP_TRY(ctx, hipGetLastError());
  return MSM377_OK;
}

template <class CV, class BP = CV>
int enqueue_windows(msm377_ctx* ctx, const uint32_t* d_scalars, uint64_t n_scalars, uint32_t wb, int slot, const Phase& ph) {
  const LaunchRecord k = launch_record(ctx, ph, n_scalars, wb, slot, curve_dims<CV, BP>());
  hipStream_t st = ctx->stream;
  ctx->last.stage.valid = false;
  ctx->zc.active = ph.zc_out && ph.back && ctx->knobs.zc_out && slot == 0 && !k.plan.table;
  if (ctx->zc.active) ctx->zc.out_seq++;
  if (ph.front) {
    hipLaunchKernelGGL(k_clear_words, dim3(1), dim3(256), 0, st, k.work_hist, META_BLOCK_WORDS, (uint32_t*)k.d_err, ph.clear_err ? 1u : 0u);
    int rc = enqueue_decompose(ctx, k, d_scalars);
    if (rc == MSM377_OK) rc = enqueue_sort(ctx, k);
    if (rc == MSM377_OK) rc = enqueue_accumulate<CV, BP>(ctx, k);
    if (rc) return rc;
  } else if (ph.clear_err)
    hipLaunchKernelGGL(k_clear_words, dim3(1), dim3(256), 0, st, (uint32_t*)k.d_err, 1u, (uint32_t*)nullptr, 0u);
  if (!ph.back) return MSM377_OK;
  if (ctx->capture) HIP_TRY(ctx, hipMemcpyAsync(ctx->d_buckets_snap, ctx->d_buckets, (size_t)k.slots * k.cv.bkt_words * k.buckets * 4, hipMemcpyDeviceToDevice, st));
  const int rc = enqueue_reduce<CV>(ctx, k);
  if (rc) return rc;
  if (!ctx->zc.active) {
    HIP_TRY(ctx, hipMemcpyAsync(ctx->h_partials + (size_t)slot * SLOT_WORDS, k.d_partials, (size_t)k.wc_out * k.pp * k.cv.out_words * 4, hipMemcpyDeviceToHost, st));
    HIP_TRY(ctx, hipMemcpyAsync(ctx->h_err + slot, k.d_err, sizeof(int), hipMemcpyDeviceToHost, st));
  }
  HIP_TRY(ctx, hipEventRecord(ctx->done_ev[slot], st));
  ctx->last.n = k.n, ctx->last.glv = k.glv, ctx->last.form = k.cv.form;
  ctx->last.geom_windows = k.slots, ctx->last.geom_log = k.L;
  ctx->last.stage.valid = ctx->capture && ph.front && !ph.into && wb == 0 && (k.cv.form != MSM377_STAGE_FORM_ED || ctx->capture == 2);
  return MSM377_OK;
}

int wait_zero_copy_out(msm377_ctx* ctx) {
  const auto t0 = std::chrono::steady_clock::now();
  for (uint32_t spins = 0; __atomic_load_n(&ctx->zc.h_flag[0], __ATOMIC_ACQUIRE) != ctx->zc.out_seq; spins++) {
    __builtin_ia32_pause();
    if ((spins & 0xfff) == 0xfff && std::chrono::steady_clock::now() - t0 > std::chrono::milliseconds(50)) {
      HIP_TRY(ctx, hipEventSynchronize(ctx->done_ev[0]));
      break;
    }
  }
  if (__atomic_load_n(&ctx->zc.h_flag[0], __ATOMIC_ACQUIRE) != ctx->zc.out_seq) {
    ctx->err = "zero-copy output: the window records did not arrive";
    return MSM377_EHIP;
  }
  ctx->h_err[0] = (int)__atomic_load_n(&ctx->zc.h_flag[1], __ATOMIC_RELAXED);
  return MSM377_OK;
}

int wait_windows(msm377_ctx* ctx, int slot) {
  if (ctx->zc.active && slot == 0) {
    const int rc = wait_zero_copy_out(ctx);
    if (rc || !ctx->timing) return rc;
  }
  HIP_TRY(ctx, hipEventSynchronize(ctx->done_ev[slot]));
  return MSM377_OK;
}

int collect_windows(msm377_ctx* ctx, int slot) {
  if (ctx->timing) {
    for (int s = 0; s < MSM377_NUM_STAGES; s++) {
      if (s == MSM377_STAGE_TAIL) continue;
      if (ctx->timing == 2 && s != MSM377_STAGE_ACC_KERNEL) {
        ctx->last.stage_ms[s] = 0.0;
        continue;
      }
      float ms = 0.f;
      ctx->last.stage_ms[s] = hipEventElapsedTime(&ms, ctx->ev[s][0], ctx->ev[s][1]) == hipSuccess ? ms : 0.0;
    }
    (void)hipGetLastError();
  }
  if (ctx->h_err[slot] & ERR_SCALAR) {
    ctx->err = "a scalar overflows the signed 16-bit window recode (final carry)";
    return MSM377_ESCALAR;
  }
  return MSM377_OK;
}

inline bool use_glv(const msm377_ctx* ctx) { return ctx->knobs.glv_mode == 1; }

int convert_bases_g1(msm377_ctx* ctx, const uint32_t* d_raw, uint64_t n, bool glv) {
  if (!glv) return convert_bases<G1Dev>(ctx, d_raw, n);
  if (n == 0) return MSM377_OK;
  if (ctx->timing == 1) (void)hipEventRecord(ctx->ev[MSM377_STAGE_CONVERT][0], ctx->stream2);
  hipLaunchKernelGGL(k_clear_words, dim3(1), dim3(256), 0, ctx->stream2, (uint32_t*)(ctx->d_err + 2), 1u, (uint32_t*)nullptr, 0u);
  hipLaunchKernelGGL(k_convert_bases_glv, dim3((unsigned)((n + 255) / 256)), dim3(256), 0, ctx->stream2, d_raw, ctx->d_bases, n);
  HIP_TRY(ctx, hipGetLastError());
  note_bases(ctx, MSM377_BASES_WEIERSTRASS, ctx->d_bases, n, 0, true);
  if (ctx->timing == 1) (void)hipEventRecord(ctx->ev[MSM377_STAGE_CONVERT][1], ctx->stream2);
  HIP_TRY(ctx, hipEventRecord(ctx->bases_ready, ctx->stream2));
  return MSM377_OK;
}

enum TableForm { TABLE_XYZZ = 0, TABLE_XYZZ_GLV = 1, TABLE_TE = 2, TABLE_TE_AFFINE = 3, TABLE_TE_PRECOMP = 4 };
inline bool form_is_te(int form) { return form == TABLE_TE || form == TABLE_TE_AFFINE || form == TABLE_TE_PRECOMP; }
constexpr int RC_TE_FALLBACK = 1;

inline int resident_form(const msm377_ctx* ctx, uint64_t n) {
  return (ctx->resident.form == TABLE_XYZZ_GLV && n != ctx->resident.n) ? TABLE_XYZZ : ctx->resident.form;
}
inline bool wide_table(const ResidentBases& r) { return r.form == TABLE_TE_PRECOMP && r.windows == WIDE_WINDOWS; }
inline int weierstrass_form(const msm377_ctx* ctx) { return use_glv(ctx) ? TABLE_XYZZ_GLV : TABLE_XYZZ; }
inline int pick_form(const msm377_ctx* ctx) { return ctx->knobs.g1_form == 1 ? TABLE_TE : weierstrass_form(ctx); }

int convert_table(msm377_ctx* ctx, const uint32_t* d_raw, uint64_t n, int form) {
  if (form == TABLE_TE) return convert_bases<TeDev>(ctx, d_raw, n);
  if (form == TABLE_TE_AFFINE) {
    const int rc = affine_convert_begin(ctx, d_raw, n);
    return rc ? rc : affine_convert_finish(ctx, ctx->d_bases, n);
  }
  return convert_bases_g1(ctx, d_raw, n, form == TABLE_XYZZ_GLV);
}

int run_tail(msm377_ctx* ctx, const WindowPlan& plan, const uint32_t* partials, uint8_t* out_xy) {
  const auto t0 = std::chrono::steady_clock::now();
  int tr = TAIL_OK;
  if (plan.tail == ED_TAIL)
    tr = ed_tail(ctx, partials, out_xy, plan.short_from);
  else if (plan.tail == XYZZ_TAIL && plan.on_caller)
    g1h_combine(partials, plan.records, out_xy, plan.short_from);
  else if (plan.tail == XYZZ_TAIL)
    tr = xyzz_tail(ctx, partials, out_xy, plan.short_from, plan.records);
  else if (plan.on_caller)
    tr = teh_combine(partials, plan.records, out_xy, plan.cbits(), plan.planes(), plan.short_from) ? TAIL_EXCEPTIONAL : TAIL_OK;
  else
    tr = te_tail(ctx, partials, out_xy, plan.records, plan.cbits(), plan.planes(), plan.short_from);
  ctx->last.stage_ms[MSM377_STAGE_TAIL] = std::chrono::duration<double, std::milli>(std::chrono::steady_clock::now() - t0).count();
  if (tr != TAIL_EXCEPTIONAL) return tr;
  note_fallback(ctx, MSM377_FB_TAIL);
  return RC_TE_FALLBACK;
}

struct TailArm {
  msm377_ctx* c;
  bool armed = false;
  explicit TailArm(msm377_ctx* ctx) : c(ctx) {}
  void arm() {
    if (armed || c->knobs.tail_threads <= 1 || c->knobs.tail_spin_us <= 0) return;
    armed = true;
    c->tail_pool.prewake(c->knobs.tail_spin_us, std::min(c->knobs.tail_threads, TailPool::WORKERS + 1) - 1);
  }
  void at_start(uint64_t n) {
    if (n <= (1ull << 17)) arm();
  }
  void after_accumulation() {
    if (armed || c->knobs.tail_threads <= 1 || c->knobs.tail_spin_us <= 0) return;
    const auto t0 = std::chrono::steady_clock::now();
// ... 98 lines not shown
template <class CV>
int run_chunked_upload(msm377_ctx* ctx, const uint8_t* points, const uint8_t* scalars, uint64_t n, const WindowPlan& plan) {
  constexpr size_t PB = CV::RAW_WORDS * 4;
  uint64_t cut[10];
  uint32_t K = 0;
  cut[0] = 0;
  for (uint32_t c = 1; c < ctx->knobs.upload_chunks; c++) {
    const uint64_t first_end = std::max<uint64_t>(64, (n * ctx->knobs.upload_split_pct / 100) & ~63ull);
    const uint64_t b = c == 1 ? first_end : (first_end + (n - first_end) * (c - 1) / (ctx->knobs.upload_chunks - 1)) & ~63ull;
    if (b > cut[K] && b < n) cut[++K] = b;
  }
  cut[++K] = n;
  const size_t sc_stage = (size_t)ctx->cap * 96;
  auto upload_chunk = [&](uint32_t c, HipFail* fail) -> int {
    const uint64_t first = cut[c], cnt = cut[c + 1] - cut[c];
    int r = h2d_staged(ctx, (uint8_t*)ctx->d_raw_scalars + first * 32, scalars + first * 32, cnt * 32, sc_stage + first * 32, fail);
    if (r == MSM377_OK) r = h2d_staged(ctx, (uint8_t*)ctx->d_raw_points + first * PB, points + first * PB, cnt * PB, first * PB, fail);
    return r;
  };
  int rc = upload_chunk(0, nullptr);
  if (rc) return rc;
  int up_rc = MSM377_OK;
  HipFail up_fail;
  std::atomic<uint32_t> uploaded{1};
  std::atomic<bool> upload_done{false};
  std::thread upload([&] {
    if (hipSetDevice(ctx->device) != hipSuccess) up_rc = MSM377_EHIP;
    for (uint32_t c = 1; c < K && up_rc == MSM377_OK; c++) {
      up_rc = upload_chunk(c, &up_fail);
      if (up_rc == MSM377_OK) uploaded.store(c + 1, std::memory_order_release);
    }
    upload_done.store(true, std::memory_order_release);
  });
  for (uint32_t c = 0; c < K && rc == MSM377_OK; c++) {
    while (uploaded.load(std::memory_order_acquire) <= c && !upload_done.load(std::memory_order_acquire)) std::this_thread::yield();
    if (uploaded.load(std::memory_order_acquire) <= c) {
      rc = up_fail.record(ctx, up_rc ? up_rc : MSM377_EHIP);
      break;
    }
    const uint64_t first = cut[c], cnt = cut[c + 1] - cut[c];
    Phase ph;
    ph.clear_err = c == 0;
    ph.into = c > 0;
    ph.back = c + 1 == K;
    ph.base_first = first;
    ph.plan = plan;
    rc = convert_bases<CV>(ctx, ctx->d_raw_points + first * CV::RAW_WORDS, cnt, first, c == 0);
    if (rc == MSM377_OK) rc = enqueue_windows<CV>(ctx, ctx->d_raw_scalars + first * 8, cnt, 0, 0, ph);
  }
  upload.join();
  if (rc) (void)hipStreamSynchronize(ctx->stream);
  return rc;
}

int check_args(msm377_ctx* ctx, const void* a, const void* b, uint64_t n, bool need_a) {
  if (!ctx) return MSM377_EINVAL;
  ctx->err.clear();
  if (n > ctx->cap) {
    ctx->err = "n exceeds the context capacity";
    return MSM377_EINVAL;
  }
  if (n && ((need_a && !a) || !b)) {
    ctx->err = "null input pointer";
    return MSM377_EINVAL;
  }
  if (((uintptr_t)a & 15) || ((uintptr_t)b & 15)) {
    ctx->err = "device input pointers must be 16-byte aligned";
    return MSM377_EINVAL;
  }
  return MSM377_OK;
}

template <class CK>
int check_points_device(msm377_ctx* ctx, const void* d_points, uint64_t n, uint32_t flags, msm377_check_report* out) {
  if (!out) return MSM377_EINVAL;
  flags = check_flags_normal(flags);
  if (!flags) return MSM377_EINVAL;
  int rc = check_args(ctx, d_points, d_points, n, true);
  if (rc) return rc;
  check_report_empty(out, n);
  if (n == 0) return MSM377_OK;
  HIP_TRY(ctx, hipSetDevice(ctx->device));
  uint32_t* scratch = ctx->d_work_meta;
  static_assert(CHK_WORDS <= META_BLOCK_WORDS, "the check's counters fit the work-list block");
  uint32_t* list = (flags & MSM377_CHECK_SUBGROUP) ? ctx->d_val_idx : nullptr;
  const dim3 grid((unsigned)((n + CHK_THREADS - 1) / CHK_THREADS));
  hipLaunchKernelGGL(k_check_clear, dim3(1), dim3(64), 0, ctx->stream, scratch);
  const bool timed = ctx->timing == 1;
  {
    StageTimer t(ctx, MSM377_STAGE_CONVERT, ctx->stream);
    hipLaunchKernelGGL(k_check_curve<CK>, grid, dim3(CHK_THREADS), 0, ctx->stream, (const uint32_t*)d_points, n, (flags & MSM377_CHECK_CURVE) ? 1u : 0u, scratch, list);
  }
  if (list) {
    StageTimer t(ctx, MSM377_STAGE_ACC_KERNEL, ctx->stream);
    hipLaunchKernelGGL(k_check_subgroup<CK>, grid, dim3(CHK_THREADS), 0, ctx->stream, (const uint32_t*)d_points, scratch, (const uint32_t*)list);
  }
  HIP_TRY(ctx, hipGetLastError());
  uint32_t h[CHK_WORDS];
  HIP_TRY(ctx, hipMemcpyAsync(h, scratch, sizeof h, hipMemcpyDeviceToHost, ctx->stream));
  HIP_TRY(ctx, hipStreamSynchronize(ctx->stream));
  if (timed) {
    for (int s = 0; s < MSM377_NUM_STAGES; s++) {
      float ms = 0.f;
      const bool ran = s == MSM377_STAGE_CONVERT || (list && s == MSM377_STAGE_ACC_KERNEL);
      ctx->last.stage_ms[s] = ran && hipEventElapsedTime(&ms, ctx->ev[s][0], ctx->ev[s][1]) == hipSuccess ? ms : 0.0;
    }
  }
  out->noncanonical = h[CHK_NONCANON];
  out->off_curve = h[CHK_OFFCURVE];
  out->outside_subgroup = h[CHK_OUTSIDE];
  const uint64_t key = (uint64_t)h[CHK_FIRST] | ((uint64_t)h[CHK_FIRST + 1] << 32);
  if (key != UINT64_MAX) {
    out->first_bad = key >> 2;
    const uint32_t cls = (uint32_t)(key & 3);
    out->first_bad_reason = cls == CHK_CLASS_NONCANON ? MSM377_CHECK_CANONICAL : cls == CHK_CLASS_OFFCURVE ? MSM377_CHECK_CURVE : MSM377_CHECK_SUBGROUP;
  }
  return MSM377_OK;
}

template <class CK>
int check_points_from_host(msm377_ctx* ctx, const uint8_t* points, uint64_t n, uint32_t flags, msm377_check_report* out) {
  if (!ctx || !out || !check_flags_normal(flags)) return MSM377_EINVAL;
  ctx->err.clear();
  if (n > ctx->cap) {
    ctx->err = "n exceeds the context capacity";
    return MSM377_EINVAL;
  }
  if (n && !points) {
    ctx->err = "null input pointer";
    return MSM377_EINVAL;
  }
  static_assert(MSM377_NUM_WINDOWS * sizeof(SortElem) >= CK::CV::RAW_WORDS * 4, "d_sort_temp holds the wire points of a full context");
  if (n) {
    HIP_TRY(ctx, hipSetDevice(ctx->device));
    const int rc = h2d_staged(ctx, ctx->d_sort_temp, points, n * CK::CV::RAW_WORDS * 4, 0);
    if (rc) return rc;
  }
  return check_points_device<CK>(ctx, ctx->d_sort_temp, n, flags, out);
}

int check_base_set(msm377_ctx* ctx, const void* d_points, uint64_t n) {
  if (!ctx->knobs.base_checks) return MSM377_OK;
  const int rc = check_points_device<G1Check>(ctx, d_points, n, ctx->knobs.base_checks, &ctx->last_check);
  if (rc) return rc;
  const msm377_check_report& r = ctx->last_check;
  if (r.first_bad == UINT64_MAX) return MSM377_OK;
  const char* why = r.first_bad_reason == MSM377_CHECK_CANONICAL ? "has a coordinate that is not below p"
                    : r.first_bad_reason == MSM377_CHECK_CURVE   ? "is not on the curve"
                                                                 : "is outside the prime-order subgroup";
  ctx->err = "base set refused: point " + std::to_string(r.first_bad) + " " + why + " (" + std::to_string(r.noncanonical + r.off_curve + r.outside_subgroup) + " of " +
             std::to_string(r.checked) + " points failed)";
  return MSM377_EPOINT;
}

inline bool native_forms(const msm377_ctx* ctx) { return ctx->point_form != MSM377_POINTS_WIRE || ctx->scalar_form != MSM377_SCALARS_WIRE; }
inline size_t point_stride(const msm377_ctx* ctx) { return ctx->point_form == MSM377_POINTS_MONT_FLAG ? 104 : 96; }
enum { MASK_BASES = 0, MASK_CHECK = 1 };

int import_points(msm377_ctx* ctx, const void* d_in, uint64_t n, uint32_t* d_out, int which) {
  int rc = ensure_import_buffers(ctx, false);
  if (rc) return rc;
  uint32_t* mask = ctx->native.d_inf_mask + (size_t)which * ctx->native.mask_words();
  uint32_t* count = ctx->native.d_inf_mask + 2 * ctx->native.mask_words() + which;
  const dim3 grid((unsigned)((n + IMPORT_THREADS - 1) / IMPORT_THREADS)), block(IMPORT_THREADS);
  if (ctx->point_form == MSM377_POINTS_MONT_FLAG) {
    hipLaunchKernelGGL(k_clear_words, dim3(1), dim3(256), 0, ctx->stream, count, 1u, (uint32_t*)nullptr, 0u);
// ... 156 lines not shown
  }
  if (n == 0) {
    identity_wire(out_xy);
    return MSM377_OK;
  }
  HIP_TRY(ctx, hipSetDevice(ctx->device));
  if (native_forms(ctx)) {
    const int up = upload_native(ctx, points, n * point_stride(ctx), scalars, n * 32);
    return up ? up : g1_msm_device(ctx, ctx->native.native_points(), ctx->native.native_scalars(), n, out_xy);
  }
  ctx->resident.clear();
  const int form = pick_form(ctx);
  if (n < ctx->knobs.upload_chunk_min || form == TABLE_XYZZ_GLV || ctx->capture)
    return g1_host_flow(ctx, points, scalars, n, form, out_xy, 0, 0);
  const bool te = form == TABLE_TE;
  const WindowPlan plan = plan_whole16(ctx, te ? TE_TAIL : XYZZ_TAIL);
  int rc = te ? run_chunked_upload<TeDev>(ctx, points, scalars, n, plan) : run_chunked_upload<G1Dev>(ctx, points, scalars, n, plan);
  if (rc == MSM377_OK) rc = wait_windows(ctx, 0);
  if (rc) return rc;
  const int err = ctx->h_err[0];
  if (te && (err & ERR_TE_ANY)) {
    note_fallback(ctx, (uint32_t)(err & ERR_TE_ANY));
  } else if (geometry_refused(plan, err)) {
    ctx->fallback.geometry_reruns++;
    rc = convert_table(ctx, ctx->d_raw_points, n, form);
    if (rc == MSM377_OK) rc = g1_table_msm(ctx, ctx->d_raw_scalars, n, form, out_xy);
    if (rc != RC_TE_FALLBACK) return rc;
  } else {
    rc = collect_windows(ctx, 0);
    if (rc == MSM377_OK) rc = run_tail(ctx, plan, ctx->h_partials, out_xy);
    if (rc != RC_TE_FALLBACK) return rc;
  }
  return g1_rerun_weierstrass(ctx, ctx->d_raw_points, ctx->d_raw_scalars, n, out_xy, 0, 0);
}

int g1_msm_short_device(msm377_ctx* ctx, const void* d_points, const void* d_scalars, uint64_t n, uint32_t sbytes, uint32_t bits, uint8_t out_xy[96]) {
  if (!out_xy) return MSM377_EINVAL;
  int rc = check_args(ctx, d_points, d_scalars, n, true);
  if (rc == MSM377_OK) rc = check_short_args(ctx, sbytes, bits);
  if (rc == MSM377_OK) rc = refuse_mont_short(ctx);
  return rc ? rc : g1_device_flow(ctx, d_points, d_scalars, n, out_xy, sbytes, bits);
}

int g1_msm_short(msm377_ctx* ctx, const uint8_t* points, const uint8_t* scalars, uint64_t n, uint32_t sbytes, uint32_t bits, uint8_t out_xy[96]) {
  if (!ctx || !out_xy) return MSM377_EINVAL;
  ctx->err.clear();
  if (n > ctx->cap || (n && (!points || !scalars))) {
    ctx->err = "bad arguments";
    return MSM377_EINVAL;
  }
  int rc = check_short_args(ctx, sbytes, bits);
  if (rc == MSM377_OK) rc = refuse_mont_short(ctx);
  if (rc) return rc;
  if (n == 0) {
    identity_wire(out_xy);
    return MSM377_OK;
  }
  HIP_TRY(ctx, hipSetDevice(ctx->device));
  if (native_forms(ctx)) {
    rc = upload_native(ctx, points, n * point_stride(ctx), scalars, n * sbytes);
    return rc ? rc : g1_msm_short_device(ctx, ctx->native.native_points(), ctx->native.native_scalars(), n, sbytes, bits, out_xy);
  }
  ctx->resident.clear();
  const bool te = ctx->knobs.g1_form == 1;
  const bool affine = te && ctx->knobs.te_affine_msm && n >= ctx->knobs.affine_min_points;
  return g1_host_flow(ctx, points, scalars, n, !te ? TABLE_XYZZ : affine ? TABLE_TE_AFFINE : TABLE_TE, out_xy, sbytes, bits);
}

int scalars_width_device(msm377_ctx* ctx, const void* d_scalars, uint64_t n, uint32_t sbytes, uint32_t* bits_out) {
  if (!ctx || !bits_out) return MSM377_EINVAL;
  ctx->err.clear();
  if (sbytes != 4 && sbytes != 8 && sbytes != 16 && sbytes != 32) {
    ctx->err = "scalar_bytes must be 4, 8, 16 or 32";
    return MSM377_EINVAL;
  }
  if ((n && !d_scalars) || ((uintptr_t)d_scalars & 15)) {
    ctx->err = "the device scalars pointer must be non-null and 16-byte aligned";
    return MSM377_EINVAL;
  }
  *bits_out = 0;
  if (n == 0) return MSM377_OK;
  HIP_TRY(ctx, hipSetDevice(ctx->device));
  uint32_t* d_out = ctx->d_work_meta;
  const uint64_t nwords = n * (sbytes / 4);
  const unsigned blocks = (unsigned)std::min<uint64_t>((nwords / 4 + 255) / 256 + 1, 2048);
  hipLaunchKernelGGL(k_clear_words, dim3(1), dim3(256), 0, ctx->stream, d_out, 1u, (uint32_t*)nullptr, 0u);
  hipLaunchKernelGGL(k_scalars_width, dim3(blocks), dim3(256), 0, ctx->stream, (const uint32_t*)d_scalars, nwords, sbytes / 4, d_out);
  HIP_TRY(ctx, hipGetLastError());
  uint32_t h = 0;
  HIP_TRY(ctx, hipMemcpyAsync(&h, d_out, 4, hipMemcpyDeviceToHost, ctx->stream));
  HIP_TRY(ctx, hipStreamSynchronize(ctx->stream));
  *bits_out = h;
  return MSM377_OK;
}

namespace {
int ed_device_flow(msm377_ctx* ctx, const void* d_points, const void* d_scalars, uint64_t n, uint8_t out_xy[64], bool equal_windows) {
  HIP_TRY(ctx, hipSetDevice(ctx->device));
  ctx->resident.clear();
  int rc = convert_bases<EdDev>(ctx, (const uint32_t*)d_points, n);
  if (rc) return rc;
  TailArm arm(ctx);
  arm.at_start(n);
  Phase ph;
  ph.zc_out = true;
  ph.plan = equal_windows || ctx->capture == 1 ? plan_equal16(ED_TAIL) : plan_whole16(ctx, ED_TAIL);
  for (;;) {
    rc = enqueue_windows<EdDev>(ctx, (const uint32_t*)d_scalars, n, 0, 0, ph);
    if (rc) return rc;
    arm.after_accumulation();
    rc = wait_windows(ctx, 0);
    if (rc) return rc;
    if (geometry_refused(ph.plan, ctx->h_err[0])) {
      ctx->fallback.geometry_reruns++;
      ph.plan = next_plan(ph.plan);
      continue;
    }
    rc = collect_windows(ctx, 0);
    return rc ? rc : run_tail(ctx, ph.plan, ctx->h_partials, out_xy);
  }
}
}

int ed_msm_device(msm377_ctx* ctx, const void* d_points, const void* d_scalars, uint64_t n, uint8_t out_xy[64]) {
  if (!out_xy) return MSM377_EINVAL;
  int rc = check_args(ctx, d_points, d_scalars, n, true);
  if (rc) return rc;
  if (n == 0) {
    memset(out_xy, 0, 64);
    out_xy[32] = 1;
    return MSM377_OK;
  }
  return ed_device_flow(ctx, d_points, d_scalars, n, out_xy, false);
}

int ed_msm(msm377_ctx* ctx, const uint8_t* points, const uint8_t* scalars, uint64_t n, uint8_t out_xy[64]) {
  if (!ctx || !out_xy) return MSM377_EINVAL;
  ctx->err.clear();
  if (n > ctx->cap || (n && (!points || !scalars))) {
    ctx->err = "bad arguments";
    return MSM377_EINVAL;
  }
  if (n == 0) return ed_msm_device(ctx, nullptr, nullptr, 0, out_xy);
  HIP_TRY(ctx, hipSetDevice(ctx->device));
  ctx->resident.clear();
  if (n >= ctx->knobs.upload_chunk_min && !ctx->capture) {
    const WindowPlan plan = plan_whole16(ctx, ED_TAIL);
    int rc = run_chunked_upload<EdDev>(ctx, points, scalars, n, plan);
    if (rc == MSM377_OK) rc = wait_windows(ctx, 0);
    if (rc) return rc;
    if (geometry_refused(plan, ctx->h_err[0])) {
      ctx->fallback.geometry_reruns++;
      return ed_device_flow(ctx, ctx->d_raw_points, ctx->d_raw_scalars, n, out_xy, true);
    }
    rc = collect_windows(ctx, 0);
    return rc ? rc : run_tail(ctx, plan, ctx->h_partials, out_xy);
  }
  int rc = h2d_staged(ctx, ctx->d_raw_points, points, n * 64, 0);
  if (rc == MSM377_OK) rc = h2d_staged(ctx, ctx->d_raw_scalars, scalars, n * 32, (size_t)ctx->cap * 96);
  if (rc) return rc;
  return ed_msm_device(ctx, ctx->d_raw_points, ctx->d_raw_scalars, n, out_xy);
}

int ed_generate_bases_device(msm377_ctx* ctx, uint64_t seed, uint64_t n, void* d_points_out) {
  if (!ctx || (n && !d_points_out) || ((uintptr_t)d_points_out & 15)) return MSM377_EINVAL;
  if (n == 0) return MSM377_OK;
// ... 1086 lines not shown
```

webgpu-msm-bls12-377_amd/host/engine.py:

```python
import ctypes
import os
import sys
from typing import List, NamedTuple, Optional, Sequence, Tuple

NUM_WINDOWS = 16
WINDOW_BITS = 16
PARTIAL_POINTS = 16
POINT_WORDS = 52
ED_POINT_WORDS = 36
STAGE_FORM_XYZZ, STAGE_FORM_TE, STAGE_FORM_ED = 0, 1, 2
RECORD_POINT_WORDS = 48
WINDOW_PARTIAL_BYTES = PARTIAL_POINTS * RECORD_POINT_WORDS * 4
NUM_BUCKETS = 32768
STAGE_NAMES = ("convert", "decompose", "sort", "accumulate", "reduce", "tail", "accumulate_kernel")

OK, EINVAL, EHIP, ESCALAR, ENOMEM, ESTATE, EGLVRANGE, EEXCEPTIONAL, EPOINT = 0, -1, -2, -3, -4, -5, -6, -7, -8
CHECK_CANONICAL, CHECK_CURVE, CHECK_SUBGROUP, CHECK_ALL = 1, 2, 4, 7
FB_ACCUMULATE, FB_MERGE, FB_TREE, FB_TAIL, FB_CONVERT = 4, 8, 16, 32, 64
GLV_WINDOWS = 8
POINTS_WIRE, POINTS_MONT, POINTS_MONT_FLAG = 0, 1, 2
SCALARS_WIRE, SCALARS_MONT = 0, 1
_POINT_FORMS = {"wire": POINTS_WIRE, "mont": POINTS_MONT, "mont_flag": POINTS_MONT_FLAG}
_SCALAR_FORMS = {"wire": SCALARS_WIRE, "mont": SCALARS_MONT}
_POINT_STRIDE = {POINTS_WIRE: 96, POINTS_MONT: 96, POINTS_MONT_FLAG: 104}
# ... 111 lines not shown
    @property
    def ok(self) -> bool:
        return self.first_bad is None


def _report(r: _CheckReportStruct) -> CheckReport:
    none = r.first_bad == 2**64 - 1
    return CheckReport(int(r.checked), int(r.noncanonical), int(r.off_curve), int(r.outside_subgroup), None if none else int(r.first_bad), int(r.first_bad_reason))


class MsmError(RuntimeError):

    def __init__(self, code: int, what: str, detail: str = ""):
        self.code = code
        msg = "%s failed: %s (%d)" % (what, _strerror(code), code)
        if detail:
            msg += ": " + detail
        super().__init__(msg)


def library_path() -> str:
    override = os.environ.get("MSM377_LIB")
    if override:
        return os.path.abspath(override)
    here = os.path.dirname(os.path.abspath(__file__))
    return os.path.normpath(os.path.join(here, "..", "csrc", "libmsm377.so"))


def load_library():
    global _LIB
    if _LIB is not None:
        return _LIB
    path = library_path()
    if not os.path.exists(path):
        raise ImportError(
            "msm377: %s is missing -- build it with `python -c 'import __graft_entry__ as g; g.build()'` "
            "or `make -C webgpu-msm-bls12-377_amd/csrc`; there is no CPU fallback" % path
        )
    if "torch" not in sys.modules and os.environ.get("MSM377_NO_TORCH_PRELOAD") != "1":
        try:
            import torch
        except Exception:
            pass
    lib = ctypes.CDLL(path)
    u8p, vp, u64, u32, i32 = ctypes.c_char_p, ctypes.c_void_p, ctypes.c_uint64, ctypes.c_uint32, ctypes.c_int
    sigs = {
        "msm377_version": (ctypes.c_char_p, []),
        "msm377_strerror": (ctypes.c_char_p, [i32]),
        "msm377_ctx_create": (i32, [i32, u64, ctypes.POINTER(vp)]),
        "msm377_ctx_destroy": (None, [vp]),
        "msm377_last_error": (ctypes.c_char_p, [vp]),
        "msm377_g1_msm": (i32, [vp, u8p, u8p, u64, vp]),
        "msm377_g1_msm_device": (i32, [vp, vp, vp, u64, vp]),
        "msm377_g1_set_bases": (i32, [vp, u8p, u64]),
        "msm377_g1_set_bases_device": (i32, [vp, vp, u64]),
        "msm377_g1_set_bases_precomputed": (i32, [vp, u8p, u64]),
        "msm377_g1_set_bases_precomputed_device": (i32, [vp, vp, u64]),
        "msm377_g1_msm_fixed_base": (i32, [vp, u8p, u64, vp]),
        "msm377_g1_msm_fixed_base_device": (i32, [vp, vp, u64, vp]),
        "msm377_g1_msm_fixed_base_batch_device": (i32, [vp, vp, u64, u32, vp]),
        "msm377_g1_window_partials_device": (i32, [vp, vp, vp, u64, u32, u32, vp]),
        "msm377_g1_window_partials_resident": (i32, [vp, vp, vp, u64, u32, u32, vp]),
        "msm377_g1_combine_partials": (i32, [vp, vp]),
        "msm377_g1_combine_partials_split": (i32, [vp, ctypes.c_uint32, vp]),
        "msm377_g1_combine_partials_ctx": (i32, [vp, vp, vp]),
        "msm377_ctx_get_fallback_info": (i32, [vp, ctypes.POINTER(u64), ctypes.POINTER(u32)]),
        "msm377_g1_glv_window_partials_device": (i32, [vp, vp, vp, u64, u32, u32, vp]),
        "msm377_g1_combine_window_partials": (i32, [vp, u32, vp]),
        "msm377_g1_generate_bases_device": (i32, [vp, u64, u64, vp]),
        "msm377_ed_msm": (i32, [vp, u8p, u8p, u64, vp]),
        "msm377_ed_msm_device": (i32, [vp, vp, vp, u64, vp]),
        "msm377_ed_generate_bases_device": (i32, [vp, u64, u64, vp]),
        "msm377_ctx_set_stage_capture": (i32, [vp, i32]),
        "msm377_g1_read_stage": (i32, [vp, u32, vp, vp, vp, vp]),
        "msm377_g1_read_stage_ex": (i32, [vp, u32, vp, vp, vp, vp, vp]),
        "msm377_g1_read_bases": (i32, [vp, vp, u64, u64, vp]),
        "msm377_g1_read_mul_table": (i32, [vp, u32, u32, vp, u64, u64, vp]),
        "msm377_g1_xyzz_to_affine": (i32, [vp, vp]),
        "msm377_g1_fold_window_partials": (i32, [vp, ctypes.c_uint32]),
        "msm377_ctx_set_glv": (i32, [vp, i32]),
        "msm377_ctx_set_g1_form": (i32, [vp, i32]),
        "msm377_ctx_set_timing": (i32, [vp, i32]),
        "msm377_ctx_get_stage_ms": (i32, [vp, vp]),
        "msm377_ctx_get_products_per_addition": (i32, [vp]),
        "msm377_ctx_set_precompute_window": (i32, [vp, i32]),
        "msm377_g1_add_points": (i32, [vp, u32, vp]),
        "msm377_ctx_reserve_host_staging": (i32, [vp]),
        "msm377_ctx_get_stage_form": (i32, [vp]),
        "msm377_ctx_set_narrow_max": (i32, [vp, u64]),
        "msm377_g1_check_points_device": (i32, [vp, vp, u64, u32, vp]),
        "msm377_g1_check_points": (i32, [vp, u8p, u64, u32, vp]),
        "msm377_ed_check_points_device": (i32, [vp, vp, u64, u32, vp]),
        "msm377_ed_check_points": (i32, [vp, u8p, u64, u32, vp]),
        "msm377_g1_check_points_host": (i32, [u8p, u64, u32, vp]),
        "msm377_ed_check_points_host": (i32, [u8p, u64, u32, vp]),
        "msm377_ctx_set_base_checks": (i32, [vp, u32]),
        "msm377_ctx_get_last_check": (i32, [vp, vp]),
        "msm377_g1_msm_short": (i32, [vp, u8p, u8p, u64, u32, u32, vp]),
        "msm377_g1_msm_short_device": (i32, [vp, vp, vp, u64, u32, u32, vp]),
        "msm377_g1_msm_fixed_base_short_device": (i32, [vp, vp, u64, u32, u32, vp]),
        "msm377_scalars_width_device": (i32, [vp, vp, u64, u32, ctypes.POINTER(u32)]),
        "msm377_scalars_width_host": (i32, [u8p, u64, u32, ctypes.POINTER(u32)]),
        "msm377_short_windows": (u32, [u32, u32]),
        "msm377_ctx_get_last_geometry": (i32, [vp, ctypes.POINTER(u32), ctypes.POINTER(u32)]),
        "msm377_ctx_get_last_sort_elem_bytes": (u32, [vp]),
        "msm377_ctx_set_input_format": (i32, [vp, u32, u32]),
        "msm377_ctx_get_input_format": (i32, [vp, ctypes.POINTER(u32), ctypes.POINTER(u32)]),
        "msm377_g1_import_points_host": (i32, [u8p, u64, u32, vp, vp]),
        "msm377_import_scalars_host": (i32, [u8p, u64, u32, vp]),
        "msm377_g1_result_to_native": (i32, [u8p, vp]),
        "msm377_g1_batch_mul_device": (i32, [vp, u8p, vp, u64, u32, vp, vp]),
        "msm377_g1_batch_mul": (i32, [vp, u8p, u8p, u64, u32, vp, vp]),
        "msm377_g1_batch_mul_host": (i32, [u8p, u8p, u64, u32, vp, vp]),
        "msm377_g1_batch_mul_multi_device": (i32, [vp, u8p, u32, vp, u64, u64, u64, u32, vp, vp]),
        "msm377_g1_batch_mul_multi": (i32, [vp, u8p, u32, u8p, u64, u64, u64, u32, vp, vp]),
        "msm377_g1_batch_mul_multi_host": (i32, [u8p, u32, u8p, u64, u64, u64, u32, vp, vp]),
        "msm377_ctx_get_mul_multi_table_builds": (u64, [vp]),
        "msm377_g1_set_generators": (i32, [vp, u8p, u32, i32]),
        "msm377_ctx_get_generators": (i32, [vp, vp, vp]),
        "msm377_g1_commit_rows_device": (i32, [vp, vp, u64, u32, u64, u64, u32, vp, vp]),
        "msm377_g1_commit_rows": (i32, [vp, u8p, u64, u32, u64, u64, u32, vp, vp]),
        "msm377_g1_commit_rows_host": (i32, [u8p, u32, u8p, u32, u64, u64, u64, u32, vp, vp]),
        "msm377_commit_rows_plan": (None, [u32, vp, vp, vp]),
        "msm377_g1_batch_mul_var_device": (i32, [vp, vp, vp, u64, u32, u32, vp, vp]),
        "msm377_g1_batch_mul_var": (i32, [vp, u8p, u8p, u64, u32, u32, vp, vp]),
        "msm377_g1_batch_mul_var_host": (i32, [u8p, u32, u8p, u32, u64, u32, u32, vp, vp]),
        "msm377_g1_batch_lincomb2_device": (i32, [vp, vp, vp, vp, vp, u64, u32, u32, u32, vp, vp]),
        "msm377_g1_batch_lincomb2": (i32, [vp, u8p, u8p, u8p, u8p, u64, u32, u32, u32, vp, vp]),
        "msm377_g1_batch_lincomb2_host": (i32, [u8p, u8p, u32, u8p, u8p, u32, u64, u32, u32, u32, vp, vp]),
        "msm377_ed_batch_mul_multi_device": (i32, [vp, u8p, u32, vp, u64, u64, u64, vp]),
        "msm377_ed_batch_mul_multi": (i32, [vp, u8p, u32, u8p, u64, u64, u64, vp]),
        "msm377_ed_batch_mul_multi_host": (i32, [u8p, u32, u8p, u64, u64, u64, vp]),
        "msm377_ed_ctx_get_mul_table_builds": (u64, [vp]),
        "msm377_ed_read_mul_table": (i32, [vp, u32, vp, u64, u64, vp]),
        "msm377_ctx_set_mul_window": (i32, [vp, i32]),
        "msm377_ctx_get_last_mul_window": (i32, [vp]),
        "msm377_ctx_get_mul_table_builds": (u64, [vp]),
    }
    for name, (res, args) in sigs.items():
        fn = getattr(lib, name)
        fn.restype = res
        fn.argtypes = args
    _LIB = lib
    return lib


def _strerror(code: int) -> str:
    try:
        return load_library().msm377_strerror(code).decode()
    except Exception:
        return "error"


def _check_host(fn: str, points: bytes, point_bytes: int, flags: int) -> CheckReport:
    if len(points) % point_bytes:
        raise ValueError("points buffer length must be a multiple of %d" % point_bytes)
    lib = load_library()
    rep = _CheckReportStruct()
    rc = getattr(lib, fn)(bytes(points), len(points) // point_bytes, int(flags), ctypes.addressof(rep))
    if rc:
        raise MsmError(rc, fn)
    return _report(rep)


def check_points_host(points: bytes, flags: int = CHECK_ALL) -> CheckReport:
    return _check_host("msm377_g1_check_points_host", points, 96, flags)
# ... 624 lines not shown
        import numpy as np

        raw = _StageInfoStruct()
        self._check(self._lib.msm377_g1_read_stage_ex(self._ctx, int(slot), ctypes.addressof(raw), None, None, None, None), "msm377_g1_read_stage_ex")
        w = int(raw.slots)
        info = StageInfo(w, int(raw.bucket_log), int(raw.columns), int(raw.digit_bytes), int(raw.row_ptr_len), int(raw.bucket_records), int(raw.form),
                         int(raw.table_stride), int(raw.geometry_reruns), tuple(raw.bias[:w]), tuple(raw.key_unsigned[:w]), tuple(raw.key_max[:w]))
        bufs = {
            "digits": np.empty(info.columns, dtype=np.uint32 if info.digit_bytes == 4 else np.uint16),
            "row_ptr": np.empty(info.row_ptr_len, dtype=np.uint32),
            "val_idx": np.empty(info.columns, dtype=np.uint32),
            "buckets": np.empty((info.bucket_records, ED_POINT_WORDS if info.form == STAGE_FORM_ED else POINT_WORDS), dtype=np.uint32),
        }
        res = {k: v for k, v in bufs.items() if k in want}
        if res:
            ptr = [res[k].ctypes.data if k in res else None for k in ("digits", "row_ptr", "val_idx", "buckets")]
            self._check(self._lib.msm377_g1_read_stage_ex(self._ctx, int(slot), None, *ptr), "msm377_g1_read_stage_ex")
        return info, res

    def read_stage(self, slot: int, n: int, want=("digits", "row_ptr", "val_idx", "buckets")):
        import numpy as np

        res = {}
        digits = np.empty(n, dtype=np.uint16) if "digits" in want else None
        row_ptr = np.empty(NUM_BUCKETS + 2, dtype=np.uint32) if "row_ptr" in want else None
        val_idx = np.empty(n, dtype=np.uint32) if "val_idx" in want else None
        buckets = np.empty((NUM_BUCKETS, POINT_WORDS), dtype=np.uint32) if "buckets" in want else None

        def ptr(a):
            return a.ctypes.data if a is not None else None

        self._check(self._lib.msm377_g1_read_stage(self._ctx, int(slot), ptr(digits), ptr(row_ptr), ptr(val_idx), ptr(buckets)), "msm377_g1_read_stage")
        for k, v in (("digits", digits), ("row_ptr", row_ptr), ("val_idx", val_idx), ("buckets", buckets)):
            if v is not None:
                res[k] = v
        return res

    def read_bases(self, first: int = 0, count=None, info_only: bool = False):
        import numpy as np

        raw = _BasesInfoStruct()
        self._check(self._lib.msm377_g1_read_bases(self._ctx, ctypes.addressof(raw), 0, 0, None), "msm377_g1_read_bases")
        bits = tuple(raw.window_bits[: raw.windows]) if raw.windows > 1 else ()
        info = BasesInfo(int(raw.form), int(raw.record_words), int(raw.limbs), int(raw.coords), int(raw.n), int(raw.windows), int(raw.glv), int(raw.window_stride),
                         int(raw.records), int(raw.flagged), bits)
        if info_only:
            return info, None
        count = info.records - int(first) if count is None else int(count)
        words = np.empty((count, info.record_words), dtype=np.uint32)
        self._check(self._lib.msm377_g1_read_bases(self._ctx, None, int(first), count, words.ctypes.data if count else None), "msm377_g1_read_bases")
        return info, words

    def read_mul_table(self, which="single", index: int = 0, first: int = 0, count=None, info_only: bool = False):
        import numpy as np

        w = _MUL_TABLES.get(which, which)
        raw = _MulTableInfoStruct()
        self._check(self._lib.msm377_g1_read_mul_table(self._ctx, int(w), int(index), ctypes.addressof(raw), 0, 0, None), "msm377_g1_read_mul_table")
        info = MulTableInfo(int(raw.width), int(raw.rows), int(raw.records), bytes(raw.key))
        if info_only:
            return info, None
        count = info.records - int(first) if count is None else int(count)
        words = np.empty((count, MUL_TABLE_RECORD_WORDS), dtype=np.uint32)
        self._check(self._lib.msm377_g1_read_mul_table(self._ctx, int(w), int(index), None, int(first), count, words.ctypes.data if count else None), "msm377_g1_read_mul_table")
        return info, words

    def stage_form(self) -> int:
        return int(self._lib.msm377_ctx_get_stage_form(self._ctx))

    def set_narrow_max(self, max_points: int = 1 << 16):
        self._check(self._lib.msm377_ctx_set_narrow_max(self._ctx, int(max_points)), "msm377_ctx_set_narrow_max")

    def set_g1_form(self, form="edwards"):
        f = {"edwards": 1, "weierstrass": 0}.get(form, form)
        self._check(self._lib.msm377_ctx_set_g1_form(self._ctx, int(f)), "msm377_ctx_set_g1_form")

    def set_glv(self, mode="auto"):
        m = 2 if mode == "auto" else int(mode)
        self._check(self._lib.msm377_ctx_set_glv(self._ctx, m), "msm377_ctx_set_glv")

    def set_timing(self, enabled=True):
        self._check(self._lib.msm377_ctx_set_timing(self._ctx, 2 if enabled == 2 else int(bool(enabled))), "msm377_ctx_set_timing")

    def stage_ms(self) -> dict:
        arr = (ctypes.c_double * len(STAGE_NAMES))()
        self._check(self._lib.msm377_ctx_get_stage_ms(self._ctx, ctypes.addressof(arr)), "msm377_ctx_get_stage_ms")
        return dict(zip(STAGE_NAMES, list(arr)))


    def accumulate_products(self) -> int:
        return int(self._lib.msm377_ctx_get_products_per_addition(self._ctx))


def _check_lengths(points: bytes, scalars: bytes, point_bytes: int = 96) -> int:
    if len(scalars) % 32:
        raise ValueError("scalars buffer length must be a multiple of 32")
    n = len(scalars) // 32
    if len(points) != point_bytes * n:
        raise ValueError("points buffer must hold %d bytes (%d per scalar), got %d" % (point_bytes * n, point_bytes, len(points)))
    return n
```

Baseline: 2.298.

## Drop per-MSM metadata clear kernel, default to packed sort elements, add accumulate stamps

Removes the front k_clear_words launch on steady-state calls. The zeroing of the work-list histogram, cursors, counters, key_max and the error word moves into kernels that already run (work_hist, work_scatter, merge_split_rows), using a double-buffered error slot and a dirty flag. It also makes packed 4-byte sort elements the default, with a larger LDS cache for that path. It adds device wall-clock stamping of the accumulate kernel for timing mode 2. The aim is to cut one launch per MSM and reduce sort memory traffic, at the cost of subtler state invariants across calls.

After: 2.305. No clear change (+0.3%).

```diff
diff --git a/include/msm377.h b/include/msm377.h
--- a/include/msm377.h
+++ b/include/msm377.h
@@ -247,6 +247,9 @@
 #define MSM377_STAGE_ACC_KERNEL 6
 #define MSM377_NUM_STAGES 7
 int msm377_ctx_set_timing(msm377_ctx* ctx, int enabled);
+int msm377_ctx_read_acc_stamps(msm377_ctx* ctx, uint64_t out[5]);
+uint64_t msm377_ctx_get_front_clears(const msm377_ctx* ctx);
+int msm377_ctx_mark_front_dirty(msm377_ctx* ctx);
 int msm377_ctx_get_stage_ms(msm377_ctx* ctx, double* ms_out);
 int msm377_ctx_get_products_per_addition(const msm377_ctx* ctx);
 
diff --git a/webgpu-msm-bls12-377_amd/csrc/capi.hip b/webgpu-msm-bls12-377_amd/csrc/capi.hip
--- a/webgpu-msm-bls12-377_amd/csrc/capi.hip
+++ b/webgpu-msm-bls12-377_amd/csrc/capi.hip
@@ -398,6 +398,22 @@
   return MSM377_OK;
 }
 
+int msm377_ctx_read_acc_stamps(msm377_ctx* ctx, uint64_t out[5]) {
+  if (!ctx || !out) return MSM377_EINVAL;
+  HIP_TRY(ctx, hipSetDevice(ctx->device));
+  HIP_TRY(ctx, hipStreamSynchronize(ctx->stream));
+  HIP_TRY(ctx, hipMemcpy(out, ctx->zc.d_stamps(), 16, hipMemcpyDeviceToHost));
+  out[2] = ctx->zc.h_stamps()[0], out[3] = ctx->zc.h_stamps()[1], out[4] = ctx->zc.clock_khz;
+  return MSM377_OK;
+}
+
+uint64_t msm377_ctx_get_front_clears(const msm377_ctx* ctx) { return ctx ? ctx->front_clears : 0; }
+int msm377_ctx_mark_front_dirty(msm377_ctx* ctx) {
+  if (!ctx) return MSM377_EINVAL;
+  ctx->meta_dirty = true;
+  return MSM377_OK;
+}
+
 int msm377_ctx_get_stage_ms(msm377_ctx* ctx, double* ms_out) {
   if (!ctx || !ms_out) return MSM377_EINVAL;
   for (int s = 0; s < MSM377_NUM_STAGES; s++) ms_out[s] = ctx->last.stage_ms[s];
diff --git a/webgpu-msm-bls12-377_amd/csrc/common.hpp b/webgpu-msm-bls12-377_amd/csrc/common.hpp
--- a/webgpu-msm-bls12-377_amd/csrc/common.hpp
+++ b/webgpu-msm-bls12-377_amd/csrc/common.hpp
@@ -59,6 +59,10 @@
 MSM_HD uint32_t sort_idx_sign(SortElem4 e) { return e.v & ~(((1u << SORT_SUB_BITS) - 1u) << SORT_IDX_BITS); }
 MSM_HD uint32_t range_first_key(uint32_t rg, uint32_t shift) { return rg * (KRANGE >> shift); }
 inline uint32_t sort_elem_bytes(uint64_t columns, bool wide) { return (!wide && columns <= SORT_PACKED_MAX_COLUMNS) ? 4u : 8u; }
+#ifndef MSM377_SORT_PACKED_DEFAULT
+#define MSM377_SORT_PACKED_DEFAULT 1
+#endif
+constexpr bool SORT_PACKED_DEFAULT = MSM377_SORT_PACKED_DEFAULT != 0;
 
 struct WorkItem {
   uint32_t row;
@@ -72,6 +76,9 @@
 inline uint32_t affine_blocks(uint64_t n) { return (uint32_t)((n + AFF_BLOCK_POINTS - 1) / AFF_BLOCK_POINTS); }
 
 constexpr uint32_t ACC_FLAG_WORD = 4;
+constexpr uint32_t ACC_STAMP_WORD = 8;
+static_assert(ACC_STAMP_WORD % 2 == 0 && ACC_STAMP_WORD > ACC_FLAG_WORD && (ACC_STAMP_WORD + 4) * 4 <= 64, "two aligned 64-bit words inside the 64-byte line");
+inline double acc_stamps_ms(uint64_t start, uint64_t end, uint64_t khz) { return (khz == 0 || start == ~0ull || end <= start) ? 0.0 : (double)(end - start) / (double)khz; }
 constexpr uint32_t EVEN_FROM = 13;
 constexpr uint32_t even_offset(uint32_t w) { return 16 * w - (w > EVEN_FROM ? w - EVEN_FROM : 0u); }
 static_assert(even_offset(13) == 208 && even_offset(14) == 223 && even_offset(15) == 238 && even_offset(16) == 253, "13 x 16 + 3 x 15 = 253 bits");
diff --git a/webgpu-msm-bls12-377_amd/csrc/context.hip b/webgpu-msm-bls12-377_amd/csrc/context.hip
--- a/webgpu-msm-bls12-377_amd/csrc/context.hip
+++ b/webgpu-msm-bls12-377_amd/csrc/context.hip
@@ -121,14 +121,19 @@
        hipHostGetDevicePointer((void**)&aff.dm_flag, aff.h_flag, 0) == hipSuccess &&
        own.event(&aff.up_done, hipEventDisableTiming) == hipSuccess;
   if (ok) aff.scratch.resize(aff_blocks);
-  dalloc((void**)&ctx->d_err, 4 * sizeof(int));
+  dalloc((void**)&ctx->d_err, 8 * sizeof(int));
+  ok = ok && hipMemset(ctx->d_err, 0, 8 * sizeof(int)) == hipSuccess && hipMemset(ctx->d_work_meta, 0, (size_t)META_BLOCK_WORDS * 4) == hipSuccess;
   ok = ok && own.alloc_pinned((void**)&ctx->h_partials, (size_t)2 * SLOT_WORDS * 4, host_flags) == hipSuccess &&
        hipHostGetDevicePointer((void**)&zc.dm_partials, ctx->h_partials, 0) == hipSuccess &&
        own.alloc_pinned((void**)&zc.h_flag, 64, host_flags) == hipSuccess &&
        hipHostGetDevicePointer((void**)&zc.dm_flag, zc.h_flag, 0) == hipSuccess;
   if (ok) memset(zc.h_flag, 0, 64);
+  if (ok) *reinterpret_cast<uint64_t*>(zc.h_flag + ACC_STAMP_WORD) = ~0ull;
   dalloc((void**)&zc.d_count, 64);
   ok = ok && hipMemset(zc.d_count, 0, 64) == hipSuccess;
+  int khz = 0;
+  if (ok && hipDeviceGetAttribute(&khz, hipDeviceAttributeWallClockRate, device) == hipSuccess && khz > 0) zc.clock_khz = (uint64_t)khz;
+  (void)hipGetLastError();
   ok = ok && own.alloc_pinned((void**)&ctx->h_err, 2 * sizeof(int)) == hipSuccess;
   for (int k = 0; ok && k < 2; k++) ok = ok && own.event(&ctx->done_ev[k], hipEventDisableTiming) == hipSuccess;
   for (int s = 0; ok && s < MSM377_NUM_STAGES; s++)
diff --git a/webgpu-msm-bls12-377_amd/csrc/context.hpp b/webgpu-msm-bls12-377_amd/csrc/context.hpp
--- a/webgpu-msm-bls12-377_amd/csrc/context.hpp
+++ b/webgpu-msm-bls12-377_amd/csrc/context.hpp
@@ -132,6 +132,10 @@
   uint32_t* dm_flag = nullptr;
   uint32_t* dm_partials = nullptr;
   uint32_t* d_count = nullptr;
+  unsigned long long* d_stamps() const { return reinterpret_cast<unsigned long long*>(d_count + msm377::ACC_STAMP_WORD); }
+  unsigned long long* dm_stamps() const { return reinterpret_cast<unsigned long long*>(dm_flag + msm377::ACC_STAMP_WORD); }
+  const volatile uint64_t* h_stamps() const { return reinterpret_cast<const volatile uint64_t*>(h_flag + msm377::ACC_STAMP_WORD); }
+  uint64_t clock_khz = 0;
 };
 
 struct NativeImport {
@@ -157,6 +161,7 @@
   int form = -1;
   bool glv = false;
   int products = 0;
+  bool acc_stamped = false;
   double stage_ms[MSM377_NUM_STAGES] = {};
   StageLayout stage;
   BasesLayout bases;
@@ -195,6 +200,10 @@
   uint32_t* d_split_rows = nullptr;
   uint32_t* d_ovf = nullptr;
   int* d_err = nullptr;
+  uint32_t err_word[2] = {0, 0};
+  bool meta_dirty = false;
+  uint64_t front_clears = 0;
+  int* err_ptr(int slot, bool other = false) const { return d_err + slot + 4 * (err_word[slot] ^ (other ? 1u : 0u)); }
   uint32_t* h_partials = nullptr;
   int* h_err = nullptr;
   hipEvent_t done_ev[2] = {};
diff --git a/webgpu-msm-bls12-377_amd/csrc/kernels/accumulate.hpp b/webgpu-msm-bls12-377_amd/csrc/kernels/accumulate.hpp
--- a/webgpu-msm-bls12-377_amd/csrc/kernels/accumulate.hpp
+++ b/webgpu-msm-bls12-377_amd/csrc/kernels/accumulate.hpp
@@ -34,10 +34,11 @@
 
 __global__ void __launch_bounds__(1024) k_work_hist(const uint32_t* __restrict__ row_ptr, uint32_t L, uint32_t rows, uint32_t SEG, uint32_t* __restrict__ work_hist,
                                                    uint32_t* __restrict__ row_ovf_base, uint32_t* __restrict__ counters ,
-                                                   uint32_t* __restrict__ split_rows) {
+                                                   uint32_t* __restrict__ split_rows, uint32_t* __restrict__ key_max_done ) {
   __shared__ uint32_t lh[SEG_BINS];
   __shared__ uint32_t blk[4];
   const uint32_t tid = threadIdx.x, row = blockIdx.x * 1024 + tid;
+  if (key_max_done && blockIdx.x == 0 && tid < MSM377_NUM_WINDOWS) key_max_done[tid] = 0;
   if (tid < SEG_BINS) lh[tid] = 0;
   if (tid < 2) blk[tid] = 0;
   __syncthreads();
@@ -67,11 +68,15 @@
 
 __global__ void __launch_bounds__(1024) k_work_scatter(const uint32_t* __restrict__ row_ptr, uint32_t L, uint32_t rows, uint32_t SEG,
                                                       const uint32_t* __restrict__ work_hist, uint32_t* __restrict__ cursor, uint32_t* __restrict__ total,
-                                                      WorkItem* __restrict__ work) {
+                                                      WorkItem* __restrict__ work, uint32_t* __restrict__ counters) {
   __shared__ uint32_t lh[SEG_BINS];
   __shared__ uint32_t lbase[SEG_BINS];
   __shared__ uint32_t gh[SEG_BINS];
   const uint32_t tid = threadIdx.x, row = blockIdx.x * 1024 + tid;
+  if (blockIdx.x == 0 && tid == 0) {
+    counters[2] = counters[0];
+    counters[0] = 0, counters[1] = 0;
+  }
   if (tid < SEG_BINS) {
     lh[tid] = 0;
     gh[tid] = work_hist[tid];
@@ -108,12 +113,25 @@
   __builtin_memcpy(&o, w, sizeof(T));
 }
 
-template <class CV, int OCC, class BP = CV, int PF = 0>
+__device__ __forceinline__ void stamp_start(unsigned long long* stamps) { atomicMax(&stamps[0], ~(unsigned long long)wall_clock64()); }
+__device__ __forceinline__ void stamp_end(unsigned long long* stamps) { atomicMax(&stamps[1], (unsigned long long)wall_clock64()); }
+__device__ __forceinline__ void deliver_acc_stamps(unsigned long long* stamps, unsigned long long* host_stamps) {
+  const unsigned long long not_start = stamps[0], end = stamps[1];
+  __hip_atomic_store(&host_stamps[0], ~not_start, __ATOMIC_RELAXED, __HIP_MEMORY_SCOPE_SYSTEM);
+  __hip_atomic_store(&host_stamps[1], end, __ATOMIC_RELAXED, __HIP_MEMORY_SCOPE_SYSTEM);
+  stamps[0] = 0ull, stamps[1] = 0ull;
+}
+
+template <class CV, int OCC, class BP = CV, int PF = 0, bool STAMP = false>
 __global__ void __launch_bounds__(256, OCC) k_accumulate(const uint32_t* __restrict__ row_ptr, const uint32_t* __restrict__ val_idx,
                                                        const uint32_t* __restrict__ bases, uint32_t* __restrict__ buckets, uint64_t n,
                                                        const WorkItem* __restrict__ work, const uint32_t* __restrict__ work_total,
                                                        const uint32_t* __restrict__ row_ovf_base, uint32_t* __restrict__ ovf, uint32_t SEG,
-                                                       int* __restrict__ err, const int* __restrict__ conv_err, uint32_t into, uint64_t table_stride, uint32_t L) {
+                                                       int* __restrict__ err, const int* __restrict__ conv_err, uint32_t into, uint64_t table_stride, uint32_t L,
+                                                       unsigned long long* __restrict__ stamps) {
+  if constexpr (STAMP) {
+    if (threadIdx.x == 0) stamp_start(stamps);
+  }
   const uint32_t v = blockIdx.x * 256 + threadIdx.x;
   if (v == 0 && *conv_err) atomicOr(err, *conv_err);
   if (v >= *work_total) return;
@@ -168,6 +186,9 @@
   } else {
     store_record<CV>(ovf + (size_t)(row_ovf_base[it.row] + it.seg - 1) * CV::BKT_WORDS, acc);
   }
+  if constexpr (STAMP) {
+    if (threadIdx.x == 0) stamp_end(stamps);
+  }
 }
 
 template <class F, class K>
@@ -292,9 +313,16 @@
 __global__ void __launch_bounds__(256, 2) k_merge_split_rows_quad(const uint32_t* __restrict__ row_ptr, uint32_t* __restrict__ buckets,
                                                                   const uint32_t* __restrict__ counters, const uint32_t* __restrict__ split_rows,
                                                                   const uint32_t* __restrict__ row_ovf_base, const uint32_t* __restrict__ ovf, uint32_t SEG,
-                                                                  int* __restrict__ err, uint32_t L, uint32_t* __restrict__ host_flag, uint32_t seq) {
+                                                                  int* __restrict__ err, uint32_t L, uint32_t* __restrict__ host_flag, uint32_t seq,
+                                                                  unsigned long long* __restrict__ stamps, unsigned long long* __restrict__ host_stamps,
+                                                                  uint32_t* __restrict__ hist_and_cursors, int* __restrict__ next_err) {
   if (host_flag && blockIdx.x == 0 && threadIdx.x == 0) __hip_atomic_store(host_flag, seq, __ATOMIC_RELAXED, __HIP_MEMORY_SCOPE_SYSTEM);
-  const uint32_t count = counters[0];
+  if (stamps && blockIdx.x == 0 && threadIdx.x == 0) deliver_acc_stamps(stamps, host_stamps);
+  if (blockIdx.x == 0) {
+    for (uint32_t i = threadIdx.x; i < 2 * SEG_BINS; i += 256) hist_and_cursors[i] = 0;
+    if (threadIdx.x == 0) *next_err = 0;
+  }
+  const uint32_t count = counters[2];
   const uint32_t q = threadIdx.x & 3;
   for (uint32_t i = (blockIdx.x * 256 + threadIdx.x) >> 2; i < count; i += gridDim.x * 64) {
     const uint32_t row = split_rows[i];
diff --git a/webgpu-msm-bls12-377_amd/csrc/kernels/sort.hpp b/webgpu-msm-bls12-377_amd/csrc/kernels/sort.hpp
--- a/webgpu-msm-bls12-377_amd/csrc/kernels/sort.hpp
+++ b/webgpu-msm-bls12-377_amd/csrc/kernels/sort.hpp
@@ -194,13 +194,18 @@
   }
 }
 
-constexpr uint32_t LS_CACHE = 6144;
-constexpr uint32_t LS_REG = LS_CACHE / 256;
+#ifndef MSM377_LS_CACHE_PACKED
+#define MSM377_LS_CACHE_PACKED 8192
+#endif
+template <class E>
+constexpr uint32_t LS_CACHE_OF = sizeof(E) == 4 ? (uint32_t)MSM377_LS_CACHE_PACKED : 6144u;
+static_assert(MSM377_LS_CACHE_PACKED % 256 == 0 && MSM377_LS_CACHE_PACKED >= 256 && MSM377_LS_CACHE_PACKED <= 12288, "whole elements per thread; `sorted` fits 64 KB of LDS with room to spare");
 template <class E>
 __global__ void __launch_bounds__(256) k_local_sort_lds(const E* __restrict__ temp, const uint32_t* __restrict__ region_base,
                                                         uint32_t* __restrict__ row_ptr, uint32_t* __restrict__ val_idx, uint64_t n,
                                                         const uint32_t* __restrict__ key_max, uint32_t NR, uint32_t NBK) {
   using Ops = ElemOps<E>;
+  constexpr uint32_t LS_CACHE = LS_CACHE_OF<E>, LS_REG = LS_CACHE / 256;
   constexpr uint32_t NBINS = KRANGE + 1;
   static_assert(NBINS <= 256, "one bin per thread");
   __shared__ uint32_t bins[NBINS];
diff --git a/webgpu-msm-bls12-377_amd/csrc/knobs.hpp b/webgpu-msm-bls12-377_amd/csrc/knobs.hpp
--- a/webgpu-msm-bls12-377_amd/csrc/knobs.hpp
+++ b/webgpu-msm-bls12-377_amd/csrc/knobs.hpp
@@ -40,6 +40,8 @@
   bool reduce_columns = true;
   bool even_windows = true;
   uint32_t sort_elem = 8;
+  bool sort_elem_env = false;
+  bool packed_sort_wanted() const { return sort_elem_env ? sort_elem == 4 : SORT_PACKED_DEFAULT; }
   bool twin_batches = true;
   uint32_t base_checks = 0;
   uint32_t tail_from = 7;
@@ -61,7 +63,7 @@
 template <auto F>
 void i64(Knobs& k, const char* e) { k.*F = atoll(e); }
 inline void wide_or_16(Knobs& k, const char* e) { k.precomp_bits = atoi(e) == (int)WIDE_BITS ? (int)WIDE_BITS : MSM377_WINDOW_BITS; }
-inline void four_or_8(Knobs& k, const char* e) { k.sort_elem = atoi(e) == 4 ? 4u : 8u; }
+inline void four_or_8(Knobs& k, const char* e) { k.sort_elem = atoi(e) == 4 ? 4u : 8u, k.sort_elem_env = true; }
 inline void check_mask(Knobs& k, const char* e) { k.base_checks = check_flags_normal((uint32_t)strtoul(e, nullptr, 0)); }
 }
 
diff --git a/webgpu-msm-bls12-377_amd/csrc/sequencer.hip b/webgpu-msm-bls12-377_amd/csrc/sequencer.hip
--- a/webgpu-msm-bls12-377_amd/csrc/sequencer.hip
+++ b/webgpu-msm-bls12-377_amd/csrc/sequencer.hip
@@ -118,8 +118,9 @@
   msm377_ctx* c;
   int s;
   hipStream_t st;
-  bool on() const { return c->timing == 1 || (c->timing == 2 && s == MSM377_STAGE_ACC_KERNEL); }
-  StageTimer(msm377_ctx* ctx, int stage, hipStream_t stream) : c(ctx), s(stage), st(stream) {
+  bool stamped;
+  bool on() const { return c->timing == 1 || (c->timing == 2 && s == MSM377_STAGE_ACC_KERNEL && !stamped); }
+  StageTimer(msm377_ctx* ctx, int stage, hipStream_t stream, bool stamped_launch = false) : c(ctx), s(stage), st(stream), stamped(stamped_launch) {
     if (on()) (void)hipEventRecord(c->ev[s][0], st);
   }
   ~StageTimer() {
@@ -327,6 +328,7 @@
   uint32_t coop_from, tail_from;
   size_t tail_lds_bytes;
   int* d_err;
+  int* next_err;
   uint32_t* d_partials;
   const uint32_t* bases;
   uint32_t *work_hist, *cursor, *total, *counters;
@@ -347,11 +349,11 @@
   k.rows = k.slots * k.buckets, k.max_items = (uint64_t)k.rows + k.entries / k.SEG;
   k.wc_out = plan.table ? 1u : k.slots, k.pp = k.wide ? WIDE_POINTS : (uint32_t)MSM377_G1_PARTIAL_POINTS;
   k.quad_acc = cv.quad_items && k.narrow && !plan.table && k.max_items <= ctx->knobs.narrow_quad_items;
-  k.packed_sort = !k.wide && !k.narrow && ctx->knobs.sort_elem == 4 && sort_elem_bytes(k.n, false) == 4;
+  k.packed_sort = !k.wide && !k.narrow && ctx->knobs.packed_sort_wanted() && sort_elem_bytes(k.n, false) == 4;
   for (k.coop_from = 0; k.coop_from < k.L && 4ull * (k.coop_from + 1) * (k.buckets >> (k.coop_from + 1)) * k.wc_out > ctx->knobs.coop_threads;) k.coop_from++;
   k.tail_from = std::min(k.wide ? k.L - 8 : k.narrow ? ctx->knobs.narrow_tail_from : ctx->knobs.tail_from, k.L);
   k.tail_lds_bytes = (size_t)(k.buckets >> k.tail_from) * cv.pt_words * 4;
-  k.d_err = ctx->d_err + slot, k.d_partials = ctx->d_partials + (size_t)slot * SLOT_WORDS;
+  k.d_err = ctx->err_ptr(slot), k.next_err = ctx->err_ptr(slot, true), k.d_partials = ctx->d_partials + (size_t)slot * SLOT_WORDS;
   const uint32_t* records = ctx->resident.valid() ? ctx->resident.bases : ctx->d_bases;
   k.bases = plan.table ? plan.table : plan.bases_override ? plan.bases_override : records + ph.base_first * cv.rec_words;
   k.work_hist = ctx->d_work_meta, k.cursor = k.work_hist + SEG_BINS, k.total = k.work_hist + 2 * SEG_BINS, k.counters = k.total + 1;
@@ -442,7 +444,9 @@
 
 template <class CV, class BP>
 void launch_accumulate(msm377_ctx* ctx, const LaunchRecord& k) {
-  StageTimer tk(ctx, MSM377_STAGE_ACC_KERNEL, ctx->stream);
+  const bool stamped = ctx->timing == 2 && !k.quad_acc && ctx->zc.clock_khz != 0;
+  ctx->last.acc_stamped = stamped;
+  StageTimer tk(ctx, MSM377_STAGE_ACC_KERNEL, ctx->stream, stamped);
   hipStream_t st = ctx->stream;
   if constexpr (curve_dims<CV, BP>().quad_items) {
     if (k.quad_acc) {
@@ -451,8 +455,9 @@
       return;
     }
   }
-  hipLaunchKernelGGL((k_accumulate<CV, 2, BP>), dim3((unsigned)((k.max_items + 255) / 256)), dim3(256), 0, st, ctx->d_row_ptr, ctx->d_val_idx, k.bases, ctx->d_buckets, k.n,
-                     ctx->d_work, k.total, ctx->d_row_ovf_base, ctx->d_ovf, k.SEG, k.d_err, ctx->d_err + 2, k.into, k.plan.table_stride, k.L);
+  const auto kernel = stamped ? k_accumulate<CV, 2, BP, 0, true> : k_accumulate<CV, 2, BP>;
+  hipLaunchKernelGGL(kernel, dim3((unsigned)((k.max_items + 255) / 256)), dim3(256), 0, st, ctx->d_row_ptr, ctx->d_val_idx, k.bases, ctx->d_buckets, k.n,
+                     ctx->d_work, k.total, ctx->d_row_ovf_base, ctx->d_ovf, k.SEG, k.d_err, ctx->d_err + 2, k.into, k.plan.table_stride, k.L, ctx->zc.d_stamps());
 }
 
 template <class CV, class BP>
@@ -460,9 +465,10 @@
   StageTimer t(ctx, MSM377_STAGE_ACCUMULATE, ctx->stream);
   hipStream_t st = ctx->stream;
   const dim3 row_grid((k.rows + 1023) / 1024);
-  hipLaunchKernelGGL(k_work_hist, row_grid, dim3(1024), 0, st, ctx->d_row_ptr, k.L, k.rows, k.SEG, k.work_hist, ctx->d_row_ovf_base, k.counters, ctx->d_split_rows);
+  hipLaunchKernelGGL(k_work_hist, row_grid, dim3(1024), 0, st, ctx->d_row_ptr, k.L, k.rows, k.SEG, k.work_hist, ctx->d_row_ovf_base, k.counters, ctx->d_split_rows,
+                     ctx->capture ? nullptr : k.key_max);
   HIP_TRY(ctx, hipGetLastError());
-  hipLaunchKernelGGL(k_work_scatter, row_grid, dim3(1024), 0, st, ctx->d_row_ptr, k.L, k.rows, k.SEG, (const uint32_t*)k.work_hist, k.cursor, k.total, ctx->d_work);
+  hipLaunchKernelGGL(k_work_scatter, row_grid, dim3(1024), 0, st, ctx->d_row_ptr, k.L, k.rows, k.SEG, (const uint32_t*)k.work_hist, k.cursor, k.total, ctx->d_work, k.counters);
   HIP_TRY(ctx, hipGetLastError());
   if (ctx->before_accumulate) {
     std::function<int()> f;
@@ -480,7 +486,8 @@
     HIP_TRY(ctx, hipGetLastError());
   }
   hipLaunchKernelGGL(k_merge_split_rows_quad<CV>, dim3(std::min<uint32_t>((k.rows + 63) / 64, 1024u)), dim3(256), 0, st, ctx->d_row_ptr, ctx->d_buckets, k.counters,
-                     ctx->d_split_rows, ctx->d_row_ovf_base, ctx->d_ovf, k.SEG, k.d_err, k.L, ctx->zc.dm_flag + ACC_FLAG_WORD, ctx->zc.acc_seq);
+                     ctx->d_split_rows, ctx->d_row_ovf_base, ctx->d_ovf, k.SEG, k.d_err, k.L, ctx->zc.dm_flag + ACC_FLAG_WORD, ctx->zc.acc_seq,
+                     ctx->last.acc_stamped ? ctx->zc.d_stamps() : nullptr, ctx->zc.dm_stamps(), k.work_hist, k.next_err);
   HIP_TRY(ctx, hipGetLastError());
   return MSM377_OK;
 }
@@ -531,17 +538,24 @@
 
 template <class CV, class BP = CV>
 int enqueue_windows(msm377_ctx* ctx, const uint32_t* d_scalars, uint64_t n_scalars, uint32_t wb, int slot, const Phase& ph) {
+  const bool dirty = ctx->meta_dirty;
+  if (ph.front && ph.clear_err && !dirty) ctx->err_word[slot] ^= 1u;
   const LaunchRecord k = launch_record(ctx, ph, n_scalars, wb, slot, curve_dims<CV, BP>());
   hipStream_t st = ctx->stream;
   ctx->last.stage.valid = false;
   ctx->zc.active = ph.zc_out && ph.back && ctx->knobs.zc_out && slot == 0 && !k.plan.table;
   if (ctx->zc.active) ctx->zc.out_seq++;
   if (ph.front) {
-    hipLaunchKernelGGL(k_clear_words, dim3(1), dim3(256), 0, st, k.work_hist, META_BLOCK_WORDS, (uint32_t*)k.d_err, ph.clear_err ? 1u : 0u);
+    ctx->meta_dirty = true;
+    if (dirty) {
+      hipLaunchKernelGGL(k_clear_words, dim3(1), dim3(256), 0, st, k.work_hist, META_BLOCK_WORDS, (uint32_t*)k.d_err, ph.clear_err ? 1u : 0u);
+      ctx->front_clears++;
+    }
     int rc = enqueue_decompose(ctx, k, d_scalars);
     if (rc == MSM377_OK) rc = enqueue_sort(ctx, k);
     if (rc == MSM377_OK) rc = enqueue_accumulate<CV, BP>(ctx, k);
     if (rc) return rc;
+    ctx->meta_dirty = ctx->capture != 0;
   } else if (ph.clear_err)
     hipLaunchKernelGGL(k_clear_words, dim3(1), dim3(256), 0, st, (uint32_t*)k.d_err, 1u, (uint32_t*)nullptr, 0u);
   if (!ph.back) return MSM377_OK;
@@ -591,6 +605,10 @@
       if (s == MSM377_STAGE_TAIL) continue;
       if (ctx->timing == 2 && s != MSM377_STAGE_ACC_KERNEL) {
         ctx->last.stage_ms[s] = 0.0;
+        continue;
+      }
+      if (ctx->timing == 2 && ctx->last.acc_stamped) {
+        ctx->last.stage_ms[s] = acc_stamps_ms(ctx->zc.h_stamps()[0], ctx->zc.h_stamps()[1], ctx->zc.clock_khz);
         continue;
       }
       float ms = 0.f;
@@ -855,6 +873,7 @@
   if (n == 0) return MSM377_OK;
   HIP_TRY(ctx, hipSetDevice(ctx->device));
   uint32_t* scratch = ctx->d_work_meta;
+  ctx->meta_dirty = true;
   static_assert(CHK_WORDS <= META_BLOCK_WORDS, "the check's counters fit the work-list block");
   uint32_t* list = (flags & MSM377_CHECK_SUBGROUP) ? ctx->d_val_idx : nullptr;
   const dim3 grid((unsigned)((n + CHK_THREADS - 1) / CHK_THREADS));
@@ -1177,6 +1196,7 @@
   if (n == 0) return MSM377_OK;
   HIP_TRY(ctx, hipSetDevice(ctx->device));
   uint32_t* d_out = ctx->d_work_meta;
+  ctx->meta_dirty = true;
   const uint64_t nwords = n * (sbytes / 4);
   const unsigned blocks = (unsigned)std::min<uint64_t>((nwords / 4 + 255) / 256 + 1, 2048);
   hipLaunchKernelGGL(k_clear_words, dim3(1), dim3(256), 0, ctx->stream, d_out, 1u, (uint32_t*)nullptr, 0u);
diff --git a/webgpu-msm-bls12-377_amd/host/engine.py b/webgpu-msm-bls12-377_amd/host/engine.py
--- a/webgpu-msm-bls12-377_amd/host/engine.py
+++ b/webgpu-msm-bls12-377_amd/host/engine.py
@@ -217,6 +217,9 @@
         "msm377_ctx_set_g1_form": (i32, [vp, i32]),
         "msm377_ctx_set_timing": (i32, [vp, i32]),
         "msm377_ctx_get_stage_ms": (i32, [vp, vp]),
+        "msm377_ctx_read_acc_stamps": (i32, [vp, vp]),
+        "msm377_ctx_get_front_clears": (u64, [vp]),
+        "msm377_ctx_mark_front_dirty": (i32, [vp]),
         "msm377_ctx_get_products_per_addition": (i32, [vp]),
         "msm377_ctx_set_precompute_window": (i32, [vp, i32]),
         "msm377_g1_add_points": (i32, [vp, u32, vp]),
@@ -1007,6 +1010,17 @@
     def set_timing(self, enabled=True):
         self._check(self._lib.msm377_ctx_set_timing(self._ctx, 2 if enabled == 2 else int(bool(enabled))), "msm377_ctx_set_timing")
 
+    def read_acc_stamps(self) -> dict:
+        arr = (ctypes.c_uint64 * 5)()
+        self._check(self._lib.msm377_ctx_read_acc_stamps(self._ctx, ctypes.addressof(arr)), "msm377_ctx_read_acc_stamps")
+        return {"device": (int(arr[0]), int(arr[1])), "start": int(arr[2]), "end": int(arr[3]), "khz": int(arr[4])}
+
+    def front_clears(self) -> int:
+        return int(self._lib.msm377_ctx_get_front_clears(self._ctx))
+
+    def mark_front_dirty(self):
+        self._check(self._lib.msm377_ctx_mark_front_dirty(self._ctx), "msm377_ctx_mark_front_dirty")
+
     def stage_ms(self) -> dict:
         arr = (ctypes.c_double * len(STAGE_NAMES))()
         self._check(self._lib.msm377_ctx_get_stage_ms(self._ctx, ctypes.addressof(arr)), "msm377_ctx_get_stage_ms")
```
